# tanmayrainanda/ishara

Hardware: AMD Instinct MI355X
Metric: landmark-frames/sec training (B=256,T=384,d=256) (higher is better)
Workload: dtype bf16; 1 GPU; configs[1]: get_model(dim=256, 2 squeeze + 2 conformer blocks, kernel_sizes=[11,5,3]) CTC train step (fwd+CTC+bwd+RAdam/Lookahead, dropout on); batch_per_gpu=256, global_batch=256, frames=384, features=224, params=7577784, parallelism=dp1, ranks_seen=1

## Files before the change

include/ishara_hip.h:

```cpp
#ifndef ISHARA_HIP_H
#define ISHARA_HIP_H
#include <stdint.h>
#ifdef __cplusplus
extern "C" {
#endif

typedef struct ishara_model ishara_model;
typedef void* ishara_stream;

enum { ISHARA_F32 = 0, ISHARA_BF16 = 1, ISHARA_F16 = 2 };
enum { ISHARA_FAMILY_KERAS_HYBRID = 0, ISHARA_FAMILY_TORCH_CONFORMER = 1, ISHARA_FAMILY_TORCH_SQUEEZEFORMER = 2 };

typedef struct ishara_config {
    int32_t dim;
    int32_t num_conv_squeeze_blocks;
    int32_t num_conv_conform_blocks;
    int32_t num_kernel_sizes;
    int32_t kernel_sizes[8];
    int32_t num_conv_per_block;
    float   dropout_rate;
    int32_t num_heads;
    int32_t expansion_factor;
    int32_t transformer_kernel_size;
    int32_t frames;
// ... 19 lines not shown
int  ishara_create(const ishara_config* cfg, ishara_model** out);
void ishara_destroy(ishara_model* m);

int64_t ishara_param_total(const ishara_model* m);
int64_t ishara_param_trainable(const ishara_model* m);
int32_t ishara_param_entries(const ishara_model* m);
int  ishara_param_info(const ishara_model* m, int32_t i, const char** name, int32_t* ndim,
                       int64_t shape[2], int64_t* offset, int32_t* trainable);
int64_t ishara_workspace_bytes(const ishara_model* m);

int32_t ishara_workspace_plan_check(const ishara_model* m);
int ishara_workspace_guard_check(ishara_model* m);

int ishara_bind(ishara_model* m, float* params, float* grads, float* opt_m, float* opt_v,
                float* opt_slow, void* workspace, int64_t workspace_bytes);
int ishara_sync_weights(ishara_model* m, ishara_stream s);

int ishara_forward(ishara_model* m, const float* x, int32_t B, float* logits, int32_t training,
                   uint32_t seed, ishara_stream s);
int ishara_loss_backward(ishara_model* m, const float* logits, const int64_t* labels, int32_t B,
                         float* loss, float* nll, float loss_scale, ishara_stream s);
int ishara_encoder_forward(ishara_model* m, const float* x, int32_t B, float* y, int32_t training, uint32_t seed, ishara_stream s);
int32_t ishara_encoder_output_frames(const ishara_model* m);
int ishara_encoder_backward(ishara_model* m, const float* dy, int32_t B, float* dx, ishara_stream s);
int32_t ishara_grad_buckets(const ishara_model* m);
int ishara_grad_bucket(const ishara_model* m, int32_t i, int64_t* offset, int64_t* count);
int ishara_grad_buckets_enable(ishara_model* m);
int ishara_grad_bucket_wait(ishara_model* m, int32_t i, ishara_stream side);
int ishara_optimizer_step(ishara_model* m, float lr, float weight_decay, ishara_stream s);
int32_t ishara_optimizer_iterations(const ishara_model* m);
int ishara_optimizer_set_iterations(ishara_model* m, int32_t it);

typedef struct ishara_grad_stats { float norm; float coef; int32_t nonfinite; int32_t skipped; } ishara_grad_stats;
int64_t ishara_grad_stats_workspace_bytes(int64_t n);
int ishara_gradient_stats(ishara_model* prof, const float* g, int64_t n, float grad_scale, float clip_norm, ishara_grad_stats* out, void* ws,
                          ishara_stream s);
int ishara_gradient_accumulate(ishara_model* prof, float* acc, const float* g, int64_t n, int32_t first, ishara_stream s);
int ishara_optimizer_step_ex(ishara_model* m, float lr, float weight_decay, const float* grad, ishara_grad_stats* st, int32_t skip_nonfinite,
                             ishara_stream s);

int ishara_profile_enable(ishara_model* m, int32_t on);
int ishara_profile_report(ishara_model* m, char* buf, int32_t cap);

int ishara_greedy_decode(const float* logits, int32_t B, int32_t T, int32_t C, int32_t blank,
                         int32_t* out_idx, int32_t* out_len, ishara_stream s);
int ishara_preprocess(const float* raw, const int32_t* n_frames, int32_t max_frames, const float* mean, const float* stdv,
                      float* out, int32_t T, ishara_stream s);
int ishara_preprocess_batch(const float* raw, int64_t n_total, const int64_t* offsets, int32_t B, int32_t max_frames,
                            const float* mean, const float* stdv, float* out, int32_t T, ishara_stream s);
int ishara_edit_distance(const int32_t* out_idx, const int32_t* out_len, int32_t B, int32_t T, const int32_t* targets, int32_t L,
                         int32_t* dist, int32_t* tlen, ishara_stream s);

int64_t ishara_ctc_beam_workspace_bytes(int32_t B, int32_t T, int32_t C, int32_t beam_width);
int ishara_ctc_beam_decode(const float* logits, int32_t B, int32_t T, int32_t C, int32_t blank, int32_t beam_width, int32_t nbest,
                           const float* lm, float alpha, float beta, void* workspace,
                           int32_t* out_idx, int32_t* out_len, float* out_score, ishara_stream s);

int64_t ishara_ctc_align_workspace_bytes(int32_t B, int32_t T, int32_t L);
int ishara_ctc_align(const float* logits, const int64_t* labels, int32_t B, int32_t T, int32_t C, int32_t L, int32_t blank,
                     void* ws, int32_t* frame_pos, int32_t* start, int32_t* end, float* conf, float* score, ishara_stream s);

typedef struct ishara_clip_aug {
    int64_t offset;
    int32_t n;
    int32_t L1;
    int32_t shift;
    int32_t L2;
    int32_t mirror;
    int32_t t0[3];
    int32_t t1[3];
    int32_t fingers[3];
} ishara_clip_aug;
enum { ISHARA_LAYOUT_FLAT = 0, ISHARA_LAYOUT_HANDS_LIPS_XY = 1 };
int ishara_clip_batch(const float* raw, const ishara_clip_aug* clips, int32_t B, int32_t T, int32_t layout,
                      float* x, ishara_stream s);
int64_t ishara_ctc_workspace_bytes(int32_t B, int32_t T, int32_t L);
int ishara_ctc_loss(const float* logits, const int64_t* labels, int32_t B, int32_t T, int32_t C,
                    int32_t L, int32_t blank, float* nll, float* dlogits, float grad_scale,
                    void* ws, ishara_stream s);
int ishara_dropout_mask(uint32_t seed, uint32_t site, int32_t rows, int32_t cols, float rate,
                        float* out, ishara_stream s);

int ishara_debug_set_as_flags(int32_t flags);
const char* ishara_debug_dense_kernel_name(int32_t dt, int32_t M, int32_t K, int32_t N, int32_t act, int32_t with_resid);
int ishara_debug_set_nt_big(int32_t on);
int ishara_debug_force_regstage(int32_t on);
int32_t ishara_debug_module_count(ishara_model* m);
int ishara_debug_module_info(ishara_model* m, int32_t i, const char** name, int32_t* in_cols, int32_t* out_cols, int32_t* first_site, int32_t* n_sites);
int ishara_debug_module_forward(ishara_model* m, int32_t i, const float* x, int32_t B, float* y, int32_t training, uint32_t seed, ishara_stream s);
int ishara_debug_module_backward(ishara_model* m, int32_t i, const float* dy, int32_t B, float* dx, ishara_stream s);
int ishara_debug_head_loss_backward(ishara_model* m, const float* logits, const int64_t* labels, int32_t B, float* loss, float* nll,
                                    float loss_scale, float* dx, ishara_stream s);

int64_t ishara_op_scratch_bytes(int32_t M, int32_t K, int32_t N);
int ishara_op_dense_fwd(int32_t dt, const void* x, const float* W, const float* bias, void* y,
                        int32_t M, int32_t K, int32_t N, int32_t act, void* scratch, ishara_stream s);
int ishara_op_dense_fwd_ex(int32_t dt, const void* x, const float* W, const float* bias, const void* resid, void* y,
                           int32_t M, int32_t K, int32_t N, int32_t act, void* scratch, ishara_stream s);
int ishara_op_dense_bwd(int32_t dt, const void* x, const float* W, const void* dy, void* dx,
                        float* dW, float* db, int32_t M, int32_t K, int32_t N, void* scratch, ishara_stream s);
int64_t ishara_op_qkv_scratch_bytes(int32_t B, int32_t T, int32_t H, int32_t dh);
int ishara_op_qkv_fwd(int32_t dt, const void* x, const float* gamma, const float* beta, float eps, const float* W, const float* bias,
                      void* q, void* k, void* vt, int32_t B, int32_t T, int32_t H, int32_t dh, int32_t head_major, void* scratch, ishara_stream s);
int ishara_op_classifier_fwd(int32_t dt, const void* x, const float* W, const float* bias, float* logits, int32_t M, int32_t K, int32_t C,
                             int32_t route, void* scratch, ishara_stream s);
int ishara_op_ctc_loss(const float* logits, const int64_t* labels, int32_t B, int32_t T, int32_t C, int32_t L, int32_t blank,
                       float* nll, float* dlogits, float grad_scale, void* ws, void* dlb, ishara_stream s);
int ishara_op_log_softmax_fwd(const float* x, float* y, int32_t M, int32_t C, int32_t ld, ishara_stream s);
int ishara_op_log_softmax_bwd(const float* dy, const float* y, float* dx, int32_t M, int32_t C, int32_t ld, ishara_stream s);
int ishara_op_layernorm_fwd(int32_t dt, const void* x, const float* gamma, const float* beta, float eps,
                            void* y, float* mean, float* rstd, int32_t M, int32_t C, ishara_stream s);
int ishara_op_layernorm_bwd(int32_t dt, const void* dy, const void* x, const float* mean, const float* rstd,
                            const float* gamma, void* dx, float* dgamma, float* dbeta, int32_t M, int32_t C,
                            ishara_stream s);
int ishara_op_dwconv_fwd(int32_t dt, int32_t inop, const void* x, const float* w, const float* bias, void* y,
                         float* ssum, float* ssq, int32_t B, int32_t T, int32_t C, int32_t k, int32_t padl,
                         ishara_stream s);
int64_t ishara_op_dwconv_fwd_scratch_bytes(int32_t B, int32_t T, int32_t C);
int ishara_op_dwconv_fwd_ex(int32_t dt, int32_t inop, const void* x, const float* w, const float* bias, void* y,
                            float* ssum, float* ssq, void* scratch, int32_t B, int32_t T, int32_t C, int32_t k,
                            int32_t padl, ishara_stream s);
int64_t ishara_op_dwconv_scratch_bytes(int32_t C, int32_t k);
int ishara_op_dwconv_bwd(int32_t dt, int32_t inop, const void* dy, const void* x, const float* w, void* dx,
                         float* dw, float* dbias, void* scratch, int32_t B, int32_t T, int32_t C, int32_t k,
                         int32_t padl, ishara_stream s);
int64_t ishara_op_attn_scratch_bytes(int32_t B, int32_t H, int32_t T, int32_t dh);
int ishara_op_attn_scratch_layout_bytes(int32_t B, int32_t H, int32_t T, int32_t dh, int64_t* out);
int ishara_op_attn_fwd(int32_t dt, const void* qkv, void* o, int32_t B, int32_t H, int32_t T, int32_t dh,
                       float scale, uint32_t seed, uint32_t site, float rate, int32_t impl,
                       void* scratch, ishara_stream s);
int ishara_op_attn_bwd(int32_t dt, const void* o, const void* dout, void* dqkv, int32_t B, int32_t H,
                       int32_t T, int32_t dh, float scale, uint32_t seed, uint32_t site, float rate,
                       int32_t impl, void* scratch, ishara_stream s);

int64_t ishara_op_relattn_scratch_bytes(int32_t B, int32_t H, int32_t T, int32_t dh);
int ishara_op_relattn_fwd(int32_t dt, const void* q, const void* k, const void* v, const float* pe, const float* Wpos, const float* u, const float* vb,
                          void* o, float* lse, int32_t B, int32_t H, int32_t T, int32_t dh, uint32_t seed, uint32_t site, float rate,
                          void* scratch, ishara_stream s);
int ishara_op_relattn_bwd(int32_t dt, const void* q, const void* k, const void* v, const float* u, const float* vb, const void* o, const void* dO,
                          void* dq, void* dk, void* dv, float* du, float* dvb, float* dWpos, float* dposp,
                          int32_t B, int32_t H, int32_t T, int32_t dh, uint32_t seed, uint32_t site, float rate, void* scratch, ishara_stream s);
int64_t ishara_op_r4_subsample_scratch_bytes(int32_t B, int32_t T0, int32_t F, int32_t d);
int ishara_op_r4_subsample_fwd(int32_t dt, const float* x, const float* w1, const float* b1, const float* w2, const float* b2, void* sub,
                               int32_t B, int32_t T0, int32_t F, int32_t d, void* scratch, ishara_stream s);
int ishara_op_r4_subsample_bwd(int32_t dt, const float* x, const float* w1, const float* w2, const void* sub, const void* dsub,
                               float* dw1, float* db1, float* dw2, float* db2, float* dx, int32_t B, int32_t T0, int32_t F, int32_t d,
                               void* scratch, ishara_stream s);
int64_t ishara_op_r4_time_reduce_scratch_bytes(int32_t B, int32_t Tin, int32_t d);
int ishara_op_r4_time_reduce_fwd(int32_t dt, const void* h, const float* conv_w, const float* conv_b, const float* Wred, const float* bred,
                                 void* red, void* conv_out, int32_t B, int32_t Tin, int32_t d, void* scratch, ishara_stream s);
int ishara_op_r4_time_reduce_bwd(int32_t dt, const void* h, const float* conv_w, const void* dred, const void* extra, void* dh,
                                 float* dconv_w, float* dconv_b, float* dWred, float* dbred, int32_t B, int32_t Tin, int32_t d,
                                 void* scratch, ishara_stream s);
int ishara_op_r4_rows(int32_t dt, int32_t mode, const void* src, const void* a, void* dst, int32_t B, int32_t Tdst, int32_t Tsrc, int32_t d,
                      ishara_stream s);

#ifdef __cplusplus
}
#endif
#endif
```

ishara_amd/_lib.py:

```python
from __future__ import annotations

import ctypes as C
import os

_HERE = os.path.dirname(os.path.abspath(__file__))
LIB_PATH = os.path.join(_HERE, "libishara_hip.so")

F32, BF16, F16 = 0, 1, 2
FAMILY_KERAS_HYBRID, FAMILY_TORCH_CONFORMER, FAMILY_TORCH_SQUEEZEFORMER = 0, 1, 2


class IsharaError(RuntimeError):
    pass


class Config(C.Structure):
    _fields_ = [
        ("dim", C.c_int32), ("num_conv_squeeze_blocks", C.c_int32), ("num_conv_conform_blocks", C.c_int32),
        ("num_kernel_sizes", C.c_int32), ("kernel_sizes", C.c_int32 * 8), ("num_conv_per_block", C.c_int32),
        ("dropout_rate", C.c_float), ("num_heads", C.c_int32), ("expansion_factor", C.c_int32),
        ("transformer_kernel_size", C.c_int32), ("frames", C.c_int32), ("features", C.c_int32),
        ("num_classes", C.c_int32), ("top_dim", C.c_int32), ("squeeze_expansion", C.c_int32),
        ("conformer_expansion", C.c_int32), ("head_dropout", C.c_float), ("conformer_attn_dropout", C.c_float),
        ("dtype", C.c_int32), ("max_batch", C.c_int32), ("max_label_len", C.c_int32), ("attn_impl", C.c_int32),
        ("family", C.c_int32), ("reduce_layer_index", C.c_int32), ("recover_layer_index", C.c_int32), ("half_step_residual", C.c_int32),
    ]


class ClipAug(C.Structure):
    _fields_ = [
        ("offset", C.c_int64), ("n", C.c_int32), ("L1", C.c_int32), ("shift", C.c_int32), ("L2", C.c_int32),
        ("mirror", C.c_int32), ("t0", C.c_int32 * 3), ("t1", C.c_int32 * 3), ("fingers", C.c_int32 * 3),
    ]


LAYOUT_FLAT, LAYOUT_HANDS_LIPS_XY = 0, 1


class GradStats(C.Structure):
    _fields_ = [("norm", C.c_float), ("coef", C.c_float), ("nonfinite", C.c_int32), ("skipped", C.c_int32)]


_P, _I32, _I64, _U32, _F = C.c_void_p, C.c_int32, C.c_int64, C.c_uint32, C.c_float
SIGNATURES = {
    "ishara_last_error": (C.c_char_p, []),
    "ishara_create": (C.c_int, [C.POINTER(Config), C.POINTER(_P)]),
    "ishara_destroy": (None, [_P]),
    "ishara_param_total": (_I64, [_P]),
    "ishara_param_trainable": (_I64, [_P]),
    "ishara_param_entries": (_I32, [_P]),
    "ishara_param_info": (C.c_int, [_P, _I32, C.POINTER(C.c_char_p), C.POINTER(_I32), C.POINTER(_I64 * 2), C.POINTER(_I64), C.POINTER(_I32)]),
    "ishara_workspace_bytes": (_I64, [_P]),
    "ishara_workspace_plan_check": (_I32, [_P]),
    "ishara_workspace_guard_check": (C.c_int, [_P]),
    "ishara_grad_buckets": (_I32, [_P]),
    "ishara_grad_bucket": (C.c_int, [_P, _I32, C.POINTER(C.c_int64), C.POINTER(C.c_int64)]),
    "ishara_grad_buckets_enable": (C.c_int, [_P]),
    "ishara_grad_bucket_wait": (C.c_int, [_P, _I32, _P]),
    "ishara_bind": (C.c_int, [_P, _P, _P, _P, _P, _P, _P, _I64]),
    "ishara_sync_weights": (C.c_int, [_P, _P]),
    "ishara_forward": (C.c_int, [_P, _P, _I32, _P, _I32, _U32, _P]),
    "ishara_encoder_forward": (C.c_int, [_P, _P, _I32, _P, _I32, _U32, _P]),
    "ishara_encoder_backward": (C.c_int, [_P, _P, _I32, _P, _P]),
    "ishara_encoder_output_frames": (_I32, [_P]),
    "ishara_loss_backward": (C.c_int, [_P, _P, _P, _I32, _P, _P, _F, _P]),
    "ishara_optimizer_step": (C.c_int, [_P, _F, _F, _P]),
    "ishara_optimizer_iterations": (_I32, [_P]),
    "ishara_optimizer_set_iterations": (C.c_int, [_P, _I32]),
    "ishara_grad_stats_workspace_bytes": (_I64, [_I64]),
    "ishara_gradient_stats": (C.c_int, [_P, _P, _I64, _F, _F, _P, _P, _P]),
    "ishara_gradient_accumulate": (C.c_int, [_P, _P, _P, _I64, _I32, _P]),
    "ishara_optimizer_step_ex": (C.c_int, [_P, _F, _F, _P, _P, _I32, _P]),
    "ishara_profile_enable": (C.c_int, [_P, _I32]),
    "ishara_profile_report": (C.c_int, [_P, C.c_char_p, _I32]),
    "ishara_greedy_decode": (C.c_int, [_P, _I32, _I32, _I32, _I32, _P, _P, _P]),
    "ishara_preprocess": (C.c_int, [_P, _P, _I32, _P, _P, _P, _I32, _P]),
    "ishara_preprocess_batch": (C.c_int, [_P, _I64, _P, _I32, _I32, _P, _P, _P, _I32, _P]),
    "ishara_edit_distance": (C.c_int, [_P, _P, _I32, _I32, _P, _I32, _P, _P, _P]),
    "ishara_ctc_beam_workspace_bytes": (_I64, [_I32, _I32, _I32, _I32]),
    "ishara_ctc_beam_decode": (C.c_int, [_P, _I32, _I32, _I32, _I32, _I32, _I32, _P, _F, _F, _P, _P, _P, _P, _P]),
    "ishara_ctc_align_workspace_bytes": (_I64, [_I32, _I32, _I32]),
    "ishara_ctc_align": (C.c_int, [_P, _P, _I32, _I32, _I32, _I32, _I32, _P, _P, _P, _P, _P, _P, _P]),
    "ishara_clip_batch": (C.c_int, [_P, _P, _I32, _I32, _I32, _P, _P]),
    "ishara_ctc_workspace_bytes": (_I64, [_I32, _I32, _I32]),
    "ishara_ctc_loss": (C.c_int, [_P, _P, _I32, _I32, _I32, _I32, _I32, _P, _P, _F, _P, _P]),
    "ishara_op_ctc_loss": (C.c_int, [_P, _P, _I32, _I32, _I32, _I32, _I32, _P, _P, _F, _P, _P, _P]),
    "ishara_dropout_mask": (C.c_int, [_U32, _U32, _I32, _I32, _F, _P, _P]),
    "ishara_debug_set_as_flags": (C.c_int, [_I32]),
    "ishara_debug_dense_kernel_name": (C.c_char_p, [_I32, _I32, _I32, _I32, _I32, _I32]),
    "ishara_debug_set_nt_big": (C.c_int, [_I32]),
    "ishara_debug_force_regstage": (C.c_int, [_I32]),
    "ishara_debug_module_count": (_I32, [_P]),
    "ishara_debug_module_info": (C.c_int, [_P, _I32, C.POINTER(C.c_char_p), C.POINTER(_I32), C.POINTER(_I32), C.POINTER(_I32), C.POINTER(_I32)]),
    "ishara_debug_module_forward": (C.c_int, [_P, _I32, _P, _I32, _P, _I32, _U32, _P]),
    "ishara_debug_module_backward": (C.c_int, [_P, _I32, _P, _I32, _P, _P]),
    "ishara_debug_head_loss_backward": (C.c_int, [_P, _P, _P, _I32, _P, _P, _F, _P, _P]),
    "ishara_op_scratch_bytes": (_I64, [_I32, _I32, _I32]),
    "ishara_op_dense_fwd": (C.c_int, [_I32, _P, _P, _P, _P, _I32, _I32, _I32, _I32, _P, _P]),
    "ishara_op_dense_fwd_ex": (C.c_int, [_I32, _P, _P, _P, _P, _P, _I32, _I32, _I32, _I32, _P, _P]),
    "ishara_op_dense_bwd": (C.c_int, [_I32, _P, _P, _P, _P, _P, _P, _I32, _I32, _I32, _P, _P]),
    "ishara_op_qkv_scratch_bytes": (_I64, [_I32, _I32, _I32, _I32]),
    "ishara_op_qkv_fwd": (C.c_int, [_I32, _P, _P, _P, _F, _P, _P, _P, _P, _P, _I32, _I32, _I32, _I32, _I32, _P, _P]),
    "ishara_op_classifier_fwd": (C.c_int, [_I32, _P, _P, _P, _P, _I32, _I32, _I32, _I32, _P, _P]),
    "ishara_op_log_softmax_fwd": (C.c_int, [_P, _P, _I32, _I32, _I32, _P]),
    "ishara_op_log_softmax_bwd": (C.c_int, [_P, _P, _P, _I32, _I32, _I32, _P]),
    "ishara_op_layernorm_fwd": (C.c_int, [_I32, _P, _P, _P, _F, _P, _P, _P, _I32, _I32, _P]),
    "ishara_op_layernorm_bwd": (C.c_int, [_I32, _P, _P, _P, _P, _P, _P, _P, _P, _I32, _I32, _P]),
    "ishara_op_dwconv_fwd": (C.c_int, [_I32, _I32, _P, _P, _P, _P, _P, _P, _I32, _I32, _I32, _I32, _I32, _P]),
    "ishara_op_dwconv_scratch_bytes": (_I64, [_I32, _I32]),
    "ishara_op_dwconv_fwd_scratch_bytes": (_I64, [_I32, _I32, _I32]),
    "ishara_op_dwconv_fwd_ex": (C.c_int, [_I32, _I32, _P, _P, _P, _P, _P, _P, _P, _I32, _I32, _I32, _I32, _I32, _P]),
    "ishara_op_dwconv_bwd": (C.c_int, [_I32, _I32, _P, _P, _P, _P, _P, _P, _P, _I32, _I32, _I32, _I32, _I32, _P]),
    "ishara_op_attn_scratch_bytes": (_I64, [_I32, _I32, _I32, _I32]),
    "ishara_op_attn_scratch_layout_bytes": (C.c_int, [_I32, _I32, _I32, _I32, C.POINTER(_I64)]),
    "ishara_op_attn_fwd": (C.c_int, [_I32, _P, _P, _I32, _I32, _I32, _I32, _F, _U32, _U32, _F, _I32, _P, _P]),
    "ishara_op_attn_bwd": (C.c_int, [_I32, _P, _P, _P, _I32, _I32, _I32, _I32, _F, _U32, _U32, _F, _I32, _P, _P]),
    "ishara_op_relattn_scratch_bytes": (_I64, [_I32, _I32, _I32, _I32]),
    "ishara_op_relattn_fwd": (C.c_int, [_I32] + [_P] * 9 + [_I32, _I32, _I32, _I32, _U32, _U32, _F, _P, _P]),
    "ishara_op_relattn_bwd": (C.c_int, [_I32] + [_P] * 14 + [_I32, _I32, _I32, _I32, _U32, _U32, _F, _P, _P]),
    "ishara_op_r4_subsample_scratch_bytes": (_I64, [_I32, _I32, _I32, _I32]),
    "ishara_op_r4_subsample_fwd": (C.c_int, [_I32] + [_P] * 6 + [_I32, _I32, _I32, _I32, _P, _P]),
    "ishara_op_r4_subsample_bwd": (C.c_int, [_I32] + [_P] * 10 + [_I32, _I32, _I32, _I32, _P, _P]),
    "ishara_op_r4_time_reduce_scratch_bytes": (_I64, [_I32, _I32, _I32]),
    "ishara_op_r4_time_reduce_fwd": (C.c_int, [_I32] + [_P] * 7 + [_I32, _I32, _I32, _P, _P]),
    "ishara_op_r4_time_reduce_bwd": (C.c_int, [_I32] + [_P] * 9 + [_I32, _I32, _I32, _P, _P]),
    "ishara_op_r4_rows": (C.c_int, [_I32, _I32, _P, _P, _P, _I32, _I32, _I32, _I32, _P]),
}

_lib = None


def load():
    global _lib
    if _lib is not None:
        return _lib
    if not os.path.exists(LIB_PATH):
        raise IsharaError(f"{LIB_PATH} is missing: build it with `python -m ishara_amd.build` "
                          "(hipcc --offload-arch=gfx950); there is no CPU fallback")
    lib = C.CDLL(LIB_PATH)
    for name, (res, args) in SIGNATURES.items():
        fn = getattr(lib, name)
        fn.restype = res
        fn.argtypes = args
    _lib = lib
    return lib


def check(rc: int, what: str = ""):
    if rc != 0:
        msg = load().ishara_last_error()
        raise IsharaError(f"{what} failed (rc={rc}): {msg.decode() if msg else '?'}")


def ptr(t):
    return None if t is None else C.c_void_p(t.data_ptr())


def stream():
    import torch
    return C.c_void_p(torch.cuda.current_stream().cuda_stream)


def aligned(nbytes: int, device):
    import torch
    t = torch.empty(int(nbytes) + 256, dtype=torch.uint8, device=device)
    return t, C.c_void_p(t.data_ptr() + (-t.data_ptr()) % 256)
```

ishara_amd/csrc/api_ops.hip:

```cpp
#include "model_types.h"

__global__ void dropout_mask_kernel(float* out, int rows, int cols, DropSpec d) {
    const size_t n = (size_t)rows * cols;
    for (size_t i = (size_t)blockIdx.x * blockDim.x + threadIdx.x; i < n; i += (size_t)gridDim.x * blockDim.x) {
        const uint32_t r = (uint32_t)(i / cols), c = (uint32_t)(i % cols);
        out[i] = (d.thr == 0u || rng_keep(rng_row_key(d.key, r), c, d.thr)) ? d.scale : 0.f;
    }
}
template <typename T>
__global__ void qkv_split_kernel(const T* qkv, T* q, T* k, T* vt, int B, int H, int Tn, int dh) {
    const int d = H * dh;
    const size_t n = (size_t)B * Tn * 3 * d;
    for (size_t i = (size_t)blockIdx.x * blockDim.x + threadIdx.x; i < n; i += (size_t)gridDim.x * blockDim.x) {
        const size_t m = i / (3 * d);
        const int col = (int)(i - m * 3 * d);
        const int h = col / (3 * dh), w = col - h * 3 * dh, part = w / dh, e = w - part * dh;
        const int b = (int)(m / Tn), t = (int)(m - (size_t)b * Tn);
        const T v = qkv[i];
        if (part == 0) q[((size_t)(b * H + h) * Tn + t) * dh + e] = v;
        else if (part == 1) k[((size_t)(b * H + h) * Tn + t) * dh + e] = v;
        else vt[((size_t)(b * H + h) * dh + e) * Tn + t] = v;
    }
}

// ... 83 lines not shown
    if (!(alpha == alpha && beta == beta) || alpha - alpha != 0.0f || beta - beta != 0.0f) { ishara_set_error("ishara_ctc_beam_decode: alpha and beta must be finite"); return -1; }
    if (B > 0 && (!logits || !workspace || !out_idx || !out_len || !out_score)) { ishara_set_error("ishara_ctc_beam_decode: null argument"); return -1; }
    if ((uintptr_t)workspace % 4) { ishara_set_error("ishara_ctc_beam_decode: workspace must be 4-byte aligned"); return -1; }
    return launch_ctc_beam(logits, B, T, C, blank, beam_width, nbest, lm, alpha, beta, workspace, out_idx, out_len, out_score, (hipStream_t)s);
}
extern "C" int64_t ishara_ctc_align_workspace_bytes(int32_t B, int32_t T, int32_t L) {
    if (B < 0 || T < 1 || T > 4096 || L < 1 || L > 255) return -1;
    return (int64_t)ctc_align_workspace_bytes(B, T, L);
}
extern "C" int ishara_ctc_align(const float* logits, const int64_t* labels, int32_t B, int32_t T, int32_t C, int32_t L, int32_t blank,
                                void* ws, int32_t* frame_pos, int32_t* start, int32_t* end, float* conf, float* score, ishara_stream s) {
    const char* me = "ishara_ctc_align";
    if (B < 0) { ishara_set_error("%s: B=%d < 0", me, B); return -1; }
    if (T < 1 || T > 4096) { ishara_set_error("%s: T=%d outside 1..4096", me, T); return -1; }
    if (L < 1 || L > 255) { ishara_set_error("%s: L=%d outside 1..255 (2L+1 lattice states in at most 8 registers of a 64-lane wave)", me, L); return -1; }
    if (C < 2 || C > 64) { ishara_set_error("%s: C=%d outside 2..64", me, C); return -1; }
    if (blank < 0 || blank >= C) { ishara_set_error("%s: blank %d outside 0..%d", me, blank, C - 1); return -1; }
    if (B == 0) return 0;
    if (!logits || !labels || !ws || !frame_pos || !start || !end || !conf || !score) {
        ishara_set_error("%s: null logits / labels / ws / frame_pos / start / end / conf / score", me); return -1;
    }
    if ((uintptr_t)ws % 16) { ishara_set_error("%s: ws must be 16-byte aligned", me); return -1; }
    return launch_ctc_align(logits, labels, B, T, C, L, blank, ws, frame_pos, start, end, conf, score, (hipStream_t)s);
}
extern "C" int ishara_clip_batch(const float* raw, const ishara_clip_aug* clips, int32_t B, int32_t T, int32_t layout,
                                 float* x, ishara_stream s) {
    if (B < 0 || T < 1 || T > CLIP_MAX_T) { ishara_set_error("ishara_clip_batch: B=%d T=%d unsupported (B >= 0, 1 <= T <= %d)", B, T, CLIP_MAX_T); return -1; }
    if (layout != ISHARA_LAYOUT_FLAT && layout != ISHARA_LAYOUT_HANDS_LIPS_XY) { ishara_set_error("ishara_clip_batch: unknown layout %d", layout); return -1; }
    if (B > 0 && (!clips || !x)) { ishara_set_error("ishara_clip_batch: null clips / x"); return -1; }
    if (((uintptr_t)raw | (uintptr_t)x) % 16) { ishara_set_error("ishara_clip_batch: raw and x must be 16-byte aligned"); return -1; }
    return launch_clip_batch(raw, clips, B, T, layout, x, (hipStream_t)s);
}

static bool op_dt_ok(const char* op, int dt, bool f16_ok) {
    if (dt != DT_F32 && dt != DT_BF16 && dt != DT_F16) { ishara_set_error("%s: unknown dtype %d (ISHARA_F32 = 0, ISHARA_BF16 = 1, ISHARA_F16 = 2)", op, dt); return false; }
    if (dt == DT_F16 && !f16_ok) { ishara_set_error("%s: ISHARA_F16 is inference-only (no fp16 backward kernels)", op); return false; }
    return true;
}
#define OP_DT(op, dt, f16_ok) do { if (!op_dt_ok(op, dt, f16_ok)) return -1; } while (0)
struct OpShadow {
    size_t wt, wn, slab, total; int ldt, ldn;
    OpShadow(int dt, int K, int N, int M) {
        const int bk = dt_is16(dt) ? 64 : 32;
        const size_t es = dt_size(dt);
        ldt = (int)rup(K, bk); ldn = (int)rup(N, bk);
        wt = 0;
        wn = rup(rup(N, 128) * (size_t)ldt * es, 256);
        slab = wn + rup(rup(K, 128) * (size_t)ldn * es, 256);
        total = slab + gemm_tn_slab_floats(M, K, N, dt) * sizeof(float);
    }
    int build(int dt, const float* Wm, int K, int N, char* sc, hipStream_t s) const {
        HIP_CHECK_RET(hipMemsetAsync(sc, 0, slab, s));
        return launch_make_shadow(dt, Wm, K, N, sc + wt, ldt, sc + wn, ldn, s);
    }
};
extern "C" int64_t ishara_op_scratch_bytes(int32_t M, int32_t K, int32_t N) {
    return (int64_t)OpShadow(DT_F32, K, N, M).total;
}
extern "C" int ishara_op_dense_fwd(int32_t dt, const void* x, const float* Wm, const float* bias, void* y, int32_t M, int32_t K, int32_t N, int32_t act, void* scratch, ishara_stream st) {
    OP_DT("ishara_op_dense_fwd", dt, true);
    hipStream_t s = (hipStream_t)st;
    const OpShadow sh(dt, K, N, M);
    char* sc = (char*)scratch;
    CK(sh.build(dt, Wm, K, N, sc, s));
    OpArgs no; EpiArgs ea; ea.bias = bias; ea.act = act; ea.dbg = g_dbg_epi;
    return launch_gemm_nt(dt, dt, dt, OP_NONE, x, sc + sh.wt, y, M, N, K, sh.ldt, no, ea, s);
}
extern "C" int ishara_op_dense_fwd_ex(int32_t dt, const void* x, const float* Wm, const float* bias, const void* resid, void* y,
                                      int32_t M, int32_t K, int32_t N, int32_t act, void* scratch, ishara_stream st) {
    OP_DT("ishara_op_dense_fwd_ex", dt, true);
    hipStream_t s = (hipStream_t)st;
    const OpShadow sh(dt, K, N, M);
    char* sc = (char*)scratch;
    CK(sh.build(dt, Wm, K, N, sc, s));
    OpArgs no; EpiArgs ea; ea.bias = bias; ea.act = act; ea.resid = resid; ea.dbg = g_dbg_epi;
    return launch_gemm_nt(dt, dt, dt, OP_NONE, x, sc + sh.wt, y, M, N, K, sh.ldt, no, ea, s);
}
extern "C" const char* ishara_debug_dense_kernel_name(int32_t dt, int32_t M, int32_t K, int32_t N, int32_t act, int32_t with_resid) {
    if (!op_dt_ok("ishara_debug_dense_kernel_name", dt, true) || M < 1 || K < 1 || N < 1) return "";
    const OpShadow sh(dt, K, N, M);
    const void* aligned = reinterpret_cast<const void*>(uintptr_t(256));
    EpiArgs ea; ea.bias = reinterpret_cast<const float*>(aligned); ea.act = act; ea.resid = with_resid ? aligned : nullptr; ea.dbg = g_dbg_epi;
    return gemm_nt_kernel_name(dt, dt, dt, OP_NONE, aligned, M, N, K, sh.ldt, ea);
}
extern "C" int ishara_op_dense_bwd(int32_t dt, const void* x, const float* Wm, const void* dy, void* dx, float* dW, float* db,
                                   int32_t M, int32_t K, int32_t N, void* scratch, ishara_stream st) {
    OP_DT("ishara_op_dense_bwd", dt, false);
    hipStream_t s = (hipStream_t)st;
    const OpShadow sh(dt, K, N, M);
    char* sc = (char*)scratch;
    CK(sh.build(dt, Wm, K, N, sc, s));
    OpArgs no; EpiArgs ea;
    if (dx) CK(launch_gemm_nt(dt, dt, dt, OP_NONE, dy, sc + sh.wn, dx, M, K, N, sh.ldn, no, ea, s));
    return launch_gemm_tn(dt, dt, dt, OP_NONE, OP_NONE, x, dy, dW, db, (float*)(sc + sh.slab), M, K, N, no, no, s);
}
static void qkv_scratch_layout(int B, int T, int H, int dh, size_t& xn, size_t& mean, size_t& rstd, size_t& total) {
    const int M = B * T, d = H * dh;
    xn = rup(OpShadow(DT_F32, d, 3 * d, M).total, 256);
    mean = xn + rup((size_t)M * d * 4, 256);
    rstd = mean + rup((size_t)M * 4, 256);
    total = rstd + rup((size_t)M * 4, 256);
}
extern "C" int64_t ishara_op_qkv_scratch_bytes(int32_t B, int32_t T, int32_t H, int32_t dh) {
    if (B < 1 || T < 1 || H < 1 || dh < 1) return -1;
    size_t xn, mean, rstd, total;
    qkv_scratch_layout(B, T, H, dh, xn, mean, rstd, total);
    return (int64_t)total;
}
extern "C" int ishara_op_qkv_fwd(int32_t dt, const void* x, const float* gamma, const float* beta, float eps, const float* Wm, const float* bias,
                                 void* q, void* k, void* vt, int32_t B, int32_t T, int32_t H, int32_t dh, int32_t head_major, void* scratch, ishara_stream st) {
    OP_DT("ishara_op_qkv_fwd", dt, true);
    if (B < 1 || T < 1 || H < 1 || dh < 1 || T % 8 != 0 || dh % 8 != 0 || (head_major != 0 && head_major != 1)) {
        ishara_set_error("ishara_op_qkv_fwd: B=%d T=%d H=%d dh=%d head_major=%d unsupported (T, dh multiples of 8; head_major 0 / 1)", B, T, H, dh, head_major); return -1;
    }
    const int d = H * dh, M = B * T;
    if ((gamma != nullptr) != (beta != nullptr) || (gamma && d > 512)) { ishara_set_error("ishara_op_qkv_fwd: LayerNorm needs both gamma and beta and H*dh <= 512 (H*dh=%d)", d); return -1; }
    if (!x || !Wm || !q || !k || !vt || !scratch || ((uintptr_t)x | (uintptr_t)scratch) % 16 != 0) { ishara_set_error("ishara_op_qkv_fwd: null or misaligned buffer (x, scratch: 16-byte aligned)"); return -1; }
    hipStream_t s = (hipStream_t)st;
    const OpShadow sh(dt, d, 3 * d, M);
    char* sc = (char*)scratch;
    CK(sh.build(dt, Wm, d, 3 * d, sc, s));
    OpArgs no;
    EpiArgs eq; eq.mode = EPI_QKV; eq.q = q; eq.k = k; eq.vt = vt; eq.H = H; eq.dh = dh; eq.T = T; eq.head_major = head_major;
    const void* A = x;
    if (gamma && !ln_as_prologue(dt, M, 3 * d, d, sh.ldt, gamma, beta, eps, nullptr, nullptr, nullptr, eq)) {
        size_t xn, mean, rstd, tot;
        qkv_scratch_layout(B, T, H, dh, xn, mean, rstd, tot);
        CK(launch_layernorm_fwd(dt, x, gamma, beta, eps, sc + xn, (float*)(sc + mean), (float*)(sc + rstd), M, d, s));
        A = sc + xn;
    }
    eq.bias = bias;
    return launch_gemm_nt(dt, dt, dt, OP_NONE, A, sc + sh.wt, nullptr, M, 3 * d, d, sh.ldt, no, eq, s);
}
extern "C" int ishara_op_classifier_fwd(int32_t dt, const void* x, const float* Wm, const float* bias, float* logits, int32_t M, int32_t K, int32_t C,
                                        int32_t route, void* scratch, ishara_stream st) {
    OP_DT("ishara_op_classifier_fwd", dt, true);
    if (route < CLS_AUTO || route > CLS_GEMM) { ishara_set_error("ishara_op_classifier_fwd: unknown route %d (0 auto, 1 A-stationary, 2 dense_narrow, 3 GEMM)", route); return -1; }
    if (M < 1 || K < 1 || C < 1) { ishara_set_error("ishara_op_classifier_fwd: bad shape M=%d K=%d C=%d", M, K, C); return -1; }
    const int r = route == CLS_AUTO ? cls_route_auto(dt, M, K, C) : route;
    const char* why = nullptr;
    if (r != CLS_GEMM && !dt_is16(dt)) why = "16-bit operands only";
    else if (r == CLS_AS && (C > 64 || C % 4 != 0 || (K != 256 && K != 512))) why = "C <= 64, C % 4 == 0 and K 256 / 512 only";
    else if (r == CLS_AS && g_force_regstage) why = "the A-stationary kernel is switched off (ishara_debug_force_regstage)";
    else if (r == CLS_NARROW && (C > 64 || K % 32 != 0)) why = "C <= 64 and K % 32 == 0 only";
    else if (r == CLS_GEMM && K % (dt_is16(dt) ? 8 : 4) != 0) why = "16-byte operand rows only";
    if (why) { ishara_set_error("ishara_op_classifier_fwd: route %d does not take dt=%d M=%d K=%d C=%d: %s", r, dt, M, K, C, why); return -1; }
    if (!x || !Wm || !logits || !scratch || ((uintptr_t)x | (uintptr_t)scratch) % 16 != 0) { ishara_set_error("ishara_op_classifier_fwd: null or misaligned buffer (x, scratch: 16-byte aligned)"); return -1; }
    hipStream_t s = (hipStream_t)st;
    const OpShadow sh(dt, K, C, M);
    char* sc = (char*)scratch;
    CK(sh.build(dt, Wm, K, C, sc, s));
    return classifier_fwd(nullptr, r, dt, x, sc + sh.wt, sh.ldt, bias, logits, M, K, C, s);
}
extern "C" int ishara_op_log_softmax_fwd(const float* x, float* y, int32_t M, int32_t C, int32_t ld, ishara_stream s) { return launch_log_softmax_fwd(x, y, M, C, ld, (hipStream_t)s); }
extern "C" int ishara_op_log_softmax_bwd(const float* dy, const float* y, float* dx, int32_t M, int32_t C, int32_t ld, ishara_stream s) { return launch_log_softmax_bwd(dy, y, dx, M, C, ld, (hipStream_t)s); }
extern "C" int ishara_op_layernorm_fwd(int32_t dt, const void* x, const float* gamma, const float* beta, float eps, void* y, float* mean, float* rstd, int32_t M, int32_t C, ishara_stream s) {
    OP_DT("ishara_op_layernorm_fwd", dt, true);
    return launch_layernorm_fwd(dt, x, gamma, beta, eps, y, mean, rstd, M, C, (hipStream_t)s);
}
extern "C" int ishara_op_layernorm_bwd(int32_t dt, const void* dy, const void* x, const float* mean, const float* rstd, const float* gamma, void* dx, float* dgamma, float* dbeta, int32_t M, int32_t C, ishara_stream s) {
    OP_DT("ishara_op_layernorm_bwd", dt, false);
    return launch_layernorm_bwd(dt, dy, x, mean, rstd, gamma, nullptr, dx, dgamma, dbeta, nullptr, M, C, (hipStream_t)s);
}
extern "C" int ishara_op_dwconv_fwd(int32_t dt, int32_t inop, const void* x, const float* w, const float* bias, void* y, float* ssum, float* ssq,
                                    int32_t B, int32_t T, int32_t C, int32_t k, int32_t padl, ishara_stream s) {
    OP_DT("ishara_op_dwconv_fwd", dt, true);
// ... 268 lines not shown
```

ishara_amd/csrc/gemm_cs.hip:

```cpp
#include <cstdio>
#include <cstdlib>
#include <map>
#include "common.h"
#include "kernels.h"

enum { CS_RESID = 1, CS_DROP = 8, CS_ROWSCALE = 16 };
#define CS_K 512
#define CS_N 256
#define CS_ROWS 384
#define CS_NST 8
#define CS_RING 4
#define CS_STAGE 32768
#define CS_DPW 4
#define CS_LDS (CS_RING * CS_STAGE + CS_N * 4 + 2 * CS_K * 4)
#define CS_DEFAULT_FLAGS 115
#define CS_MIN_M 49153

typedef __attribute__((ext_vector_type(4))) uint32_t cs_u32x4;

template <int N> DEVI void cs_wait_vm() { static_assert(N >= 0 && N < 64, "vmcnt is 6 bits"); asm volatile("s_waitcnt vmcnt(%0)" ::"n"(N) : "memory"); }
template <int N0, int NP> DEVI void cs_wait(bool counted, bool pout) {
    if (!counted) cs_wait_vm<0>(); else if (pout) cs_wait_vm<NP>(); else cs_wait_vm<N0>();
}
template <int OFF> DEVI cs_u32x4 cs_ld16(const void* p) {
    cs_u32x4 r;
    asm volatile("global_load_dwordx4 %0, %1, off offset:%2" : "=v"(r) : "v"(p), "n"(OFF) : "memory");
    return r;
}
DEVI void cs_pin(cs_u32x4& r) { asm volatile("" : "+v"(r)); }
DEVI void cs_mfma(bool first, f32x4& acc, const bf16x8& b, const cs_u32x4& a) {
    if (first) asm volatile("v_mfma_f32_16x16x32_bf16 %0, %1, %2, 0" : "=&v"(acc) : "v"(b), "v"(a));
    else asm volatile("v_mfma_f32_16x16x32_bf16 %0, %1, %2, %0" : "+v"(acc) : "v"(b), "v"(a));
}
DEVI int cs_swz(int r) { return (r & 2) | (((r >> 4) & 1) << 2); }
DEVI void cs_unpack(const cs_u32x4& r, float (&v)[8]) {
#pragma unroll
    for (int h = 0; h < 4; ++h) { v[2 * h] = __uint_as_float(r[h] << 16); v[2 * h + 1] = __uint_as_float(r[h] & 0xffff0000u); }
}
DEVI void cs_st_pk(bf16* p, const bf16x8& t, bool nt) {
    if (nt) __builtin_nontemporal_store(t, reinterpret_cast<bf16x8*>(p)); else *reinterpret_cast<bf16x8*>(p) = t;
}

struct CsLane {
    const bf16* bsrc[CS_DPW];
    int off0, off1;
    int wid, c, g;
};
template <int RT> struct CsRows {
    const bf16* ap[RT];
    int mrow[RT];
    cs_u32x4 a[3][RT][2];
};
template <int RT> DEVI void cs_rows_init(CsRows<RT>& r, const bf16* __restrict__ A, int M, int mw, const CsLane& L) {
#pragma unroll
    for (int i = 0; i < RT; ++i) {
        r.mrow[i] = min(mw + 16 * i + L.c, M - 1);
        r.ap[i] = A + (size_t)r.mrow[i] * CS_K + L.g * 8;
    }
}
template <int RT, int S> DEVI void cs_load_a(CsRows<RT>& r) {
#pragma unroll
    for (int i = 0; i < RT; ++i) {
        r.a[S % 3][i][0] = cs_ld16<S * 128>(r.ap[i]);
        r.a[S % 3][i][1] = cs_ld16<S * 128 + 64>(r.ap[i]);
    }
}
template <int S> DEVI void cs_issue_w(const CsLane& L, char* smem) {
#pragma unroll
    for (int t = 0; t < CS_DPW; ++t) {
        const bf16* src = L.bsrc[t];
        asm volatile("" : "+v"(src));
        __builtin_amdgcn_global_load_lds((const __attribute__((address_space(1))) void*)(src + S * 64),
                                         (__attribute__((address_space(3))) void*)(smem + (S % CS_RING) * CS_STAGE + (L.wid * CS_DPW + t) * 1024), 16, 0, 0);
    }
}
template <int RT> DEVI void cs_prefetch(CsRows<RT>& r, const CsLane& L, char* smem) {
    cs_load_a<RT, 0>(r);
    cs_load_a<RT, 1>(r);
    cs_issue_w<0>(L, smem);
    cs_issue_w<1>(L, smem);
    cs_issue_w<2>(L, smem);
}
#define CS_PREFETCH_OPS(RT) (2 * 2 * (RT) + 3 * CS_DPW)

template <int MASK, int PRO, int RT, int E, int S>
DEVI void cs_stage(CsRows<RT>& r, const CsLane& L, char* smem, const float* pq_s, f32x4 (&acc)[8][2][RT], bf16* pro_out, int M, int mw,
                   bool full, bool pout, bool nt_side) {
    constexpr int NA = 2 * RT, D = CS_DPW;
    if constexpr (S == 0) cs_wait<2 * D + E, 2 * D + E>(full, pout);
    else if constexpr (S == 1) cs_wait<2 * D + E + NA, 2 * D + E + NA + NA>(full, pout);
    else if constexpr (S <= 5) cs_wait<2 * D + NA, 2 * D + NA + 2 * NA>(full, pout);
    else if constexpr (S == 6) cs_wait<D + NA, D + NA + 2 * NA>(full, pout);
    else cs_wait<0, 2 * NA>(full, pout);
    asm volatile("s_waitcnt lgkmcnt(0)" ::: "memory");
    __builtin_amdgcn_s_barrier();
    if constexpr (S + 2 < CS_NST) cs_load_a<RT, S + 2>(r);
    if constexpr (S + 3 < CS_NST) cs_issue_w<S + 3>(L, smem);
    constexpr int B = S % 3;
#pragma unroll
    for (int i = 0; i < RT; ++i) { cs_pin(r.a[B][i][0]); cs_pin(r.a[B][i][1]); }
    if constexpr (PRO == 2) {
#pragma unroll
        for (int kt = 0; kt < 2; ++kt) {
            const float* cp = pq_s + 64 * S + 32 * kt + 8 * L.g;
            const f32x4 w0 = *reinterpret_cast<const f32x4*>(cp), w1 = *reinterpret_cast<const f32x4*>(cp + 4);
            const f32x4 b0 = *reinterpret_cast<const f32x4*>(cp + CS_K), b1 = *reinterpret_cast<const f32x4*>(cp + CS_K + 4);
            float wv[8], bv[8];
#pragma unroll
            for (int e = 0; e < 4; ++e) { wv[e] = w0[e]; wv[4 + e] = w1[e]; bv[e] = b0[e]; bv[4 + e] = b1[e]; }
#pragma unroll
            for (int i = 0; i < RT; ++i) {
                float v[8];
                cs_unpack(r.a[B][i][kt], v);
                bf16x8 t;
#pragma unroll
                for (int e = 0; e < 8; ++e) t[e] = (bf16)(v[e] * wv[e] + bv[e]);
                r.a[B][i][kt] = __builtin_bit_cast(cs_u32x4, t);
                if (pout && (full || mw + 16 * i + L.c < M))
                    cs_st_pk(pro_out + (size_t)r.mrow[i] * CS_K + L.g * 8 + 64 * S + 32 * kt, t, nt_side);
            }
        }
    }
    const char* st = smem + (S % CS_RING) * CS_STAGE;
    auto frag = [&](int q, int jj) { return *reinterpret_cast<const bf16x8*>(st + ((q >> 3) ? L.off1 : L.off0) + (32 * (q & 7) + 4 * jj) * 128); };
    bf16x8 b0 = frag(0, 0), b1 = frag(0, 1), c0 = frag(1, 0), c1 = frag(1, 1);
    if constexpr (PRO != 0) asm volatile("s_nop 1");
#pragma unroll
    for (int q = 0; q < 16; ++q) {
        const int kt = q >> 3, p = q & 7;
        bf16x8 n0 = c0, n1 = c1;
        if (q + 2 < 16) { n0 = frag(q + 2, 0); n1 = frag(q + 2, 1); }
        asm volatile("" ::: "memory");
#pragma unroll
        for (int i = 0; i < RT; ++i) {
            cs_mfma(S == 0 && q < 8, acc[p][0][i], b0, r.a[B][i][kt]);
            cs_mfma(S == 0 && q < 8, acc[p][1][i], b1, r.a[B][i][kt]);
        }
        b0 = c0; b1 = c1; c0 = n0; c1 = n1;
    }
}

template <int MASK, int PRO, int RT, int E, typename HAND>
DEVI void cs_pass(CsRows<RT>& r, const CsLane& L, bf16* __restrict__ C, int M, const EpiArgs& ea, char* smem, const float* bias_s, const float* pq_s,
                  int m_base, float rsc, int hops, HAND hand) {
    const int mw = m_base + L.wid * 16 * RT;
    const bool full = m_base + 128 * RT <= M;
    const bool pout = PRO != 0 && ea.pro_out != nullptr;
    const bool nt_side = (ea.as_flags & 2) != 0;
    constexpr bool f_resid = (MASK & CS_RESID) != 0, f_drop = (MASK & CS_DROP) != 0, f_rowscale = (MASK & CS_ROWSCALE) != 0;
    f32x4 acc[8][2][RT];
    bf16* po = reinterpret_cast<bf16*>(ea.pro_out);
    cs_stage<MASK, PRO, RT, E, 0>(r, L, smem, pq_s, acc, po, M, mw, full, pout, nt_side);
    cs_stage<MASK, PRO, RT, E, 1>(r, L, smem, pq_s, acc, po, M, mw, full, pout, nt_side);
    cs_stage<MASK, PRO, RT, E, 2>(r, L, smem, pq_s, acc, po, M, mw, full, pout, nt_side);
    cs_stage<MASK, PRO, RT, E, 3>(r, L, smem, pq_s, acc, po, M, mw, full, pout, nt_side);
    cs_stage<MASK, PRO, RT, E, 4>(r, L, smem, pq_s, acc, po, M, mw, full, pout, nt_side);
    cs_stage<MASK, PRO, RT, E, 5>(r, L, smem, pq_s, acc, po, M, mw, full, pout, nt_side);
    cs_stage<MASK, PRO, RT, E, 6>(r, L, smem, pq_s, acc, po, M, mw, full, pout, nt_side);
    cs_stage<MASK, PRO, RT, E, 7>(r, L, smem, pq_s, acc, po, M, mw, full, pout, nt_side);

    asm volatile("s_nop 15");
    size_t eoff[RT];
#pragma unroll
    for (int i = 0; i < RT; ++i) eoff[i] = (size_t)r.mrow[i] * CS_N + 8 * L.g;
    cs_u32x4 rs[RT][8];
    if constexpr (f_resid) {
        const bf16* resid = reinterpret_cast<const bf16*>(ea.resid);
#pragma unroll
        for (int i = 0; i < RT; ++i) {
            const bf16* rp = resid + eoff[i];
            rs[i][0] = cs_ld16<0>(rp);   rs[i][1] = cs_ld16<64>(rp);  rs[i][2] = cs_ld16<128>(rp); rs[i][3] = cs_ld16<192>(rp);
            rs[i][4] = cs_ld16<256>(rp); rs[i][5] = cs_ld16<320>(rp); rs[i][6] = cs_ld16<384>(rp); rs[i][7] = cs_ld16<448>(rp);
        }
    }
    asm volatile("s_waitcnt lgkmcnt(0)" ::: "memory");
    __builtin_amdgcn_s_barrier();
    hand();
    if constexpr (f_resid) {
        if (hops) cs_wait_vm<CS_PREFETCH_OPS(1)>(); else cs_wait_vm<0>();
#pragma unroll
        for (int i = 0; i < RT; ++i)
#pragma unroll
            for (int p = 0; p < 8; ++p) cs_pin(rs[i][p]);
    }
    uint32_t rk[RT];
#pragma unroll
    for (int i = 0; i < RT; ++i) rk[i] = f_drop ? rng_row_key(ea.drop.key, (uint32_t)(mw + 16 * i + L.c)) : 0u;
#pragma unroll
    for (int i = 0; i < RT; ++i) {
        const int m = mw + 16 * i + L.c;
        if (!full && m >= M) continue;
#pragma unroll
        for (int p = 0; p < 8; ++p) {
            const int n = 32 * p + 8 * L.g;
            float bias[8];
#pragma unroll
            for (int h = 0; h < 2; ++h) {
                const f32x4 bv = *reinterpret_cast<const f32x4*>(bias_s + n + 4 * h);
#pragma unroll
                for (int e = 0; e < 4; ++e) bias[4 * h + e] = bv[e];
            }
            float v[8];
            const float bsc = (f_rowscale && ea.rowscale_bias) ? rsc : 1.f;
#pragma unroll
            for (int e = 0; e < 4; ++e) { v[e] = acc[p][0][i][e] + bias[e] * bsc; v[4 + e] = acc[p][1][i][e] + bias[4 + e] * bsc; }
            if constexpr (f_drop) rng_apply<8>(rk[i], (uint32_t)n, ea.drop.thr, ea.drop.scale, v);
            if (f_rowscale && !ea.rowscale_bias) {
#pragma unroll
                for (int e = 0; e < 8; ++e) v[e] *= rsc;
            }
            if constexpr (f_resid) {
                float x[8];
                cs_unpack(rs[i][p], x);
#pragma unroll
                for (int e = 0; e < 8; ++e) v[e] += x[e];
            }
            store8(C + eoff[i] + 32 * p, v);
        }
    }
}

template <int MASK, int PRO>
__global__ __launch_bounds__(512, 1) void gemm_nt_cs_kernel(const bf16* __restrict__ A, const bf16* __restrict__ Bt, bf16* __restrict__ C, int M, int ldb, EpiArgs ea) {
    extern __shared__ __attribute__((aligned(16))) char cs_smem[];
    float* bias_s = reinterpret_cast<float*>(cs_smem + CS_RING * CS_STAGE);
    float* pq_s = bias_s + CS_N;
    const int tid = threadIdx.x, lane = tid & 63;
    const int m_base = blockIdx.x * CS_ROWS;
    const int bsm = min(m_base, M - 1) / max(ea.T, 1);
    for (int n = tid; n < CS_N; n += 512) bias_s[n] = ea.bias ? ea.bias[n] : 0.f;
    if constexpr (PRO == 2) {
        const float* c0 = ea.pa_P + (size_t)bsm * CS_K;
        const float* c1 = ea.pa_Q + (size_t)bsm * CS_K;
        for (int x = tid; x < CS_K; x += 512) { pq_s[x] = c0[x]; pq_s[CS_K + x] = c1[x]; }
    }
    float rsc = 1.f;
    if constexpr ((MASK & CS_ROWSCALE) != 0) rsc = ea.rowscale[bsm];
    __syncthreads();
    asm volatile("" : "+v"(rsc));

    CsLane L;
    L.wid = __builtin_amdgcn_readfirstlane(tid >> 6);
    L.c = lane & 15; L.g = lane >> 4;
#pragma unroll
    for (int t = 0; t < CS_DPW; ++t) {
        const int rr = (L.wid * CS_DPW + t) * 8 + (lane >> 3), p = lane & 7;
        L.bsrc[t] = Bt + (size_t)rr * ldb + ((p ^ cs_swz(rr)) << 3);
    }
    const int frow = 8 * (L.c >> 2) + (L.c & 3);
    const int sx = L.g ^ cs_swz(frow);
    L.off0 = frow * 128 + (sx << 4);
    L.off1 = frow * 128 + ((sx ^ 4) << 4);

    const bool two = m_base + 256 < M;
    CsRows<2> r1;
    CsRows<1> r2;
    cs_rows_init<2>(r1, A, M, m_base + L.wid * 32, L);
    cs_prefetch<2>(r1, L, cs_smem);
    cs_pass<MASK, PRO, 2, 0>(r1, L, C, M, ea, cs_smem, bias_s, pq_s, m_base, rsc, two ? CS_PREFETCH_OPS(1) : 0, [&]() {
        if (two) {
            cs_rows_init<1>(r2, A, M, m_base + 256 + L.wid * 16, L);
            cs_prefetch<1>(r2, L, cs_smem);
        }
    });
    if (two) cs_pass<MASK, PRO, 1, 16>(r2, L, C, M, ea, cs_smem, bias_s, pq_s, m_base + 256, rsc, 0, []() {});
}

static int cs_mask_of(const EpiArgs& ea) {
    return (ea.resid ? 1 : 0) | (ea.dact != DACT_NONE ? 2 : 0) | (ea.act != ACT_NONE ? 4 : 0) | (ea.drop.thr ? 8 : 0) | (ea.rowscale ? 16 : 0) |
           (ea.pre_out ? 32 : 0) | (ea.mode == EPI_QKV ? 64 : 0) | (ea.addtab ? 128 : 0);
}
static int cs_flags(const EpiArgs& ea) {
    static const int v = getenv("ISHARA_AS_FLAGS") ? atoi(getenv("ISHARA_AS_FLAGS")) : CS_DEFAULT_FLAGS;
    return ea.as_flags >= 0 ? ea.as_flags : (g_as_flags_override >= 0 ? g_as_flags_override : v);
}
bool gemm_nt_cs_applicable(int dtC, int M, int N, int K, int ldb, const EpiArgs& ea) {
    if (dtC != DT_BF16 || K != CS_K || N != CS_N || M < 1 || ldb < CS_K || ldb % 8 != 0) return false;
    const int flags = cs_flags(ea);
    if (!(flags & 64)) return false;
    if (ea.n_valid || ea.dbg || (ea.ldc && ea.ldc != CS_N) || ea.ln_gamma) return false;
    if (!(flags & 128) && M < CS_MIN_M) return false;
    const int mask = cs_mask_of(ea);
    if (ea.pa_P) return ea.pa_Q && ea.T > 0 && ea.T % CS_ROWS == 0 && (mask == CS_RESID || mask == (CS_RESID | CS_ROWSCALE));
    return mask == 0 || mask == CS_RESID || mask == (CS_RESID | CS_DROP);
}
const char* gemm_nt_cs_name(const EpiArgs& ea) {
    static std::map<int, std::string> names;
    const int mask = cs_mask_of(ea), pro = ea.pa_P ? 2 : 0;
    auto it = names.find(mask | pro << 8);
    if (it == names.end()) {
        char buf[64];
        snprintf(buf, sizeof buf, "gemm_nt_cs_kernel<%d,%d>", mask, pro);
        it = names.emplace(mask | pro << 8, buf).first;
    }
    return it->second.c_str();
}
template <int MASK, int PRO>
static int cs_launch(const void* A, const void* Bt, void* C, int M, int ldb, const EpiArgs& ea, hipStream_t s) {
    static int ready = 0;
    if (!ready) ready = hipFuncSetAttribute(reinterpret_cast<const void*>(gemm_nt_cs_kernel<MASK, PRO>), hipFuncAttributeMaxDynamicSharedMemorySize, CS_LDS) == hipSuccess ? 1 : -1;
    if (ready < 0) { ishara_set_error("gemm_nt_cs: %d bytes of LDS refused", CS_LDS); return -1; }
    hipLaunchKernelGGL((gemm_nt_cs_kernel<MASK, PRO>), dim3((M + CS_ROWS - 1) / CS_ROWS), dim3(512), CS_LDS, s, (const bf16*)A, (const bf16*)Bt, (bf16*)C, M, ldb, ea);
    return launch_rc();
}
int launch_gemm_nt_cs(int dtC, const void* A, const void* Bt, void* C, int M, int N, int K, int ldb, const EpiArgs& ea_in, hipStream_t s) {
    if (!gemm_nt_cs_applicable(dtC, M, N, K, ldb, ea_in)) return 1;
    EpiArgs ea = ea_in;
    ea.as_flags = cs_flags(ea_in);
    const int mask = cs_mask_of(ea);
    if (ea.pa_P) return mask == CS_RESID ? cs_launch<CS_RESID, 2>(A, Bt, C, M, ldb, ea, s) : cs_launch<CS_RESID | CS_ROWSCALE, 2>(A, Bt, C, M, ldb, ea, s);
    if (mask == 0) return cs_launch<0, 0>(A, Bt, C, M, ldb, ea, s);
    if (mask == CS_RESID) return cs_launch<CS_RESID, 0>(A, Bt, C, M, ldb, ea, s);
    return cs_launch<CS_RESID | CS_DROP, 0>(A, Bt, C, M, ldb, ea, s);
}
```

ishara_amd/csrc/gemm_nt.hip:

```cpp
#include "gemm_tile.h"

template <typename TA, typename TM, typename TC, int OP>
__global__ __launch_bounds__(256) void gemm_nt_kernel(const TA* __restrict__ A, const TM* __restrict__ Bt, TC* __restrict__ C,
                                                      int M, int N, int K, int ldb, int a_vec_ok, OpArgs oa, EpiArgs ea) {
    __shared__ __attribute__((aligned(16))) char smem[65536];
    constexpr int BK = MmaCfg<TM>::BK;
    const int tid = threadIdx.x, lane = tid & 63, wid = tid >> 6, wr = wid >> 1, wc = wid & 1;
    const int nMt = (M + 127) >> 7, nNt = (N + 127) >> 7;
    int mt, nt;
    {
        const int id = blockIdx.x;
        if ((nMt & 7) == 0) { const int xcd = id & 7, local = id >> 3; mt = (local / nNt) * 8 + xcd; nt = local % nNt; }
        else { mt = id / nNt; nt = id % nNt; }
    }
    const int m0 = mt << 7, n0 = nt << 7;
    const int nk = (K + BK - 1) / BK;

    u32x4 ra[4], rb[4];
    f32x4 acc[4][4];
#pragma unroll
    for (int i = 0; i < 4; ++i)
#pragma unroll
        for (int j = 0; j < 4; ++j) acc[i][j] = f32x4{0.f, 0.f, 0.f, 0.f};

// ... 413 lines not shown
                    if (ea.rowscale && !ea.rowscale_bias) {
#pragma unroll
                        for (int e = 0; e < 4; ++e) v[e] *= rsc;
                    }
                    if (need_aux) {
                        float a4[4];
                        if (need_res) load4t(reinterpret_cast<const TC*>(ea.aux) + rowoff + n, a4);
                        else {
#pragma unroll
                            for (int e = 0; e < 4; ++e) a4[e] = ext[j][e];
                        }
                        if (ea.dact == DACT_SWISH) {
#pragma unroll
                            for (int e = 0; e < 4; ++e) v[e] *= dswishf_(a4[e]);
                        } else {
#pragma unroll
                            for (int e = 0; e < 4; ++e) v[e] = a4[e] > 0.f ? v[e] : 0.f;
                        }
                    }
                    if (need_res) {
#pragma unroll
                        for (int e = 0; e < 4; ++e) v[e] += ext[j][e];
                    }
                    if (ea.mode == EPI_STD) {
                        store4t(C + rowoff + n, v);
                    } else {
                        int h, part, ii;
                        if (ea.head_major) { h = n / (3 * ea.dh); const int w = n - h * 3 * ea.dh; part = w / ea.dh; ii = w - part * ea.dh; }
                        else { part = n / dmodel; const int w = n - part * dmodel; h = w / ea.dh; ii = w - h * ea.dh; }
                        const int t = m - bsamp * ea.T;
                        if (part < 2) {
                            store4t(reinterpret_cast<TC*>(part == 0 ? ea.q : ea.k) + ((size_t)(bsamp * ea.H + h) * ea.T + t) * ea.dh + ii, v);
                        } else {
                            TC* dst = reinterpret_cast<TC*>(ea.vt) + ((size_t)(bsamp * ea.H + h) * ea.dh + ii) * ea.T + t;
#pragma unroll
                            for (int e = 0; e < 4; ++e) dst[(size_t)e * ea.T] = from_f<TC>(v[e]);
                        }
                    }
                }
            }
        } else if (acc[0][0][0] == 123.456f) C[0] = from_f<TC>(acc[1][3][2]);
        if (!more) break;
        tile = ntile; mt = mt2; nt = nt2; first = false;
    }
}

template <typename TM, typename TC>
static int run_nt_t(const void* A, const void* Bt, void* C, int M, int N, int K, int ldb, const EpiArgs& ea, hipStream_t s) {
    const int nMt = (M + 127) / 128, nNt = (N + 127) / 128;
    const int ntiles = nMt * nNt;
    const int grid = ntiles < 768 ? ntiles : 768;
    const bool fast = ea.addtab == nullptr && ea.pre_out == nullptr && ea.act == ACT_NONE && ea.drop.thr == 0 && ea.rowscale == nullptr &&
                      ea.dact == DACT_NONE && ea.mode == EPI_STD && ea.dbg == 0;
    if (fast && ea.resid) hipLaunchKernelGGL((gemm_nt_t_kernel<TM, TC, 2>), dim3(grid), dim3(256), 0, s, (const TM*)A, (const TM*)Bt, (TC*)C, M, N, K, ldb, ea);
    else if (fast) hipLaunchKernelGGL((gemm_nt_t_kernel<TM, TC, 1>), dim3(grid), dim3(256), 0, s, (const TM*)A, (const TM*)Bt, (TC*)C, M, N, K, ldb, ea);
    else hipLaunchKernelGGL((gemm_nt_t_kernel<TM, TC, 0>), dim3(grid), dim3(256), 0, s, (const TM*)A, (const TM*)Bt, (TC*)C, M, N, K, ldb, ea);
    return launch_rc();
}

template <typename TA, typename TM, typename TC, int OP>
static int run_nt(const void* A, const void* Bt, void* C, int M, int N, int K, int ldb, const OpArgs& oa, const EpiArgs& ea, hipStream_t s) {
    const int nMt = (M + 127) / 128, nNt = (N + 127) / 128;
    const int a_vec_ok = (((size_t)K * sizeof(TA)) % 16 == 0) && (((uintptr_t)A) % 16 == 0);
    hipLaunchKernelGGL((gemm_nt_kernel<TA, TM, TC, OP>), dim3(nMt * nNt), dim3(256), 0, s,
                       (const TA*)A, (const TM*)Bt, (TC*)C, M, N, K, ldb, a_vec_ok, oa, ea);
    return launch_rc();
}

template <typename TA, typename TM, typename TC>
static int run_nt_op(int op, const void* A, const void* Bt, void* C, int M, int N, int K, int ldb, const OpArgs& oa, const EpiArgs& ea, hipStream_t s) {
    switch (op) {
        case OP_NONE: return run_nt<TA, TM, TC, OP_NONE>(A, Bt, C, M, N, K, ldb, oa, ea, s);
        case OP_SWISH: return run_nt<TA, TM, TC, OP_SWISH>(A, Bt, C, M, N, K, ldb, oa, ea, s);
        case OP_COLAFFINE: return run_nt<TA, TM, TC, OP_COLAFFINE>(A, Bt, C, M, N, K, ldb, oa, ea, s);
        case OP_DROPMASK: return run_nt<TA, TM, TC, OP_DROPMASK>(A, Bt, C, M, N, K, ldb, oa, ea, s);
        default: ishara_set_error("gemm_nt: unsupported operand op %d", op); return -1;
    }
}

int g_force_regstage = 0;

NtRoute gemm_nt_route(int dtA, int dtM, int dtC, int op, const void* A, int M, int N, int K, int ldb, const EpiArgs& ea) {
    const bool pro = ea.ln_gamma || ea.pa_P;
    if (dtM == DT_F16) {
        if (op != OP_NONE) return NT_REFUSED;
        if (dtA == DT_F16 && g_force_regstage == 0 && (K == 256 || K == 512) && ldb % 64 == 0 && ((uintptr_t)A) % 16 == 0 && gemm_nt_as_applicable(dtC, M, N, K, ldb, ea)) return NT_AS_F16;
        if (pro) return NT_REFUSED;
        return (dtA == DT_F16 && (dtC == DT_F16 || dtC == DT_F32)) || (dtA == DT_F32 && dtC == DT_F16) ? NT_REG : NT_REFUSED;
    }
    if (pro && (op != OP_NONE || !gemm_nt_as_prologue_ok(dtA, dtM, dtC, M, N, K, ldb, ea))) return NT_REFUSED;
    if (g_force_regstage == 0 && gemm_nt_big_applicable(dtA, dtM, dtC, op, A, M, N, K, ldb, ea)) return NT_BIG;
    const int bk = dtM == DT_BF16 ? 32 : 16;
    const bool dma_ok = op == OP_NONE && dtA == dtM && K % bk == 0 && ldb % (2 * bk) == 0 && ((uintptr_t)A) % 16 == 0;
    if (dma_ok && g_force_regstage == 0 && dtM == DT_BF16 && gemm_nt_cs_applicable(dtC, M, N, K, ldb, ea)) return NT_CS;
    if (dma_ok && g_force_regstage == 0 && dtM == DT_BF16 && gemm_nt_as_applicable(dtC, M, N, K, ldb, ea)) return NT_AS;
    const bool dma_dt = (dtM == DT_F32 && dtC == DT_F32) || (dtM == DT_BF16 && (dtC == DT_BF16 || dtC == DT_F32));
    if (dma_ok && dma_dt && (g_force_regstage == 0 || g_force_regstage == 3) && N % 4 == 0 && (ea.mode != EPI_QKV || ea.dh % 4 == 0)) return NT_TILE_T;
    if (dma_ok && dma_dt && g_force_regstage != 1) return NT_GLDS;
    if (dtA == dtM && dtM == dtC && (dtM == DT_F32 || dtM == DT_BF16)) return NT_REG;
    if (dtM == DT_BF16 && op == OP_NONE && ((dtA == DT_F32 && dtC == DT_BF16) || (dtA == DT_BF16 && dtC == DT_F32))) return NT_REG;
    return NT_REFUSED;
}

int launch_gemm_nt(int dtA, int dtM, int dtC, int op, const void* A, const void* Bt, void* C,
                   int M, int N, int K, int ldb, const OpArgs& oa, const EpiArgs& ea, hipStream_t s) {
    if (M <= 0 || N <= 0 || K <= 0) { ishara_set_error("gemm_nt: bad shape %d %d %d", M, N, K); return -1; }
    if ((dt_is16(dtA) && K % 8 != 0) || (dtA == DT_F32 && K % 4 != 0) || ((uintptr_t)A) % 16 != 0) {
        ishara_set_error("gemm_nt: A rows must be 16-byte aligned (K=%d)", K); return -1;
    }
    if (ea.mode == EPI_QKV && (ea.T % 8 != 0 || N % 8 != 0 || ea.dh % 8 != 0)) {
        ishara_set_error("gemm_nt: QKV split needs T, dh multiples of 8 (T=%d dh=%d)", ea.T, ea.dh); return -1;
    }
    const bool f16m = dtM == DT_F16;
    int rc = 1;
    switch (gemm_nt_route(dtA, dtM, dtC, op, A, M, N, K, ldb, ea)) {
        case NT_REFUSED:
            if (f16m && op != OP_NONE) ishara_set_error("gemm_nt: f16 operands take no operand transform");
            else if (f16m && (ea.ln_gamma || ea.pa_P)) ishara_set_error("gemm_nt: f16 operand prologue on a shape the A-stationary kernel does not take");
            else if (f16m) ishara_set_error("gemm_nt: unsupported f16 dtype combination %d/%d/%d", dtA, dtM, dtC);
            else if (ea.ln_gamma || ea.pa_P) ishara_set_error("gemm_nt: operand prologue requested for a shape the A-stationary kernel does not take (check gemm_nt_as_prologue_ok first)");
            else ishara_set_error("gemm_nt: unsupported dtype combination %d/%d/%d op %d", dtA, dtM, dtC, op);
            return -1;
        case NT_AS_F16: rc = launch_gemm_nt_as_f16(dtC, A, Bt, C, M, N, K, ldb, ea, s); break;
        case NT_BIG: rc = launch_gemm_nt_big(dtA, dtM, dtC, op, A, Bt, C, M, N, K, ldb, ea, s); break;
        case NT_CS: rc = launch_gemm_nt_cs(dtC, A, Bt, C, M, N, K, ldb, ea, s); break;
        case NT_AS: rc = launch_gemm_nt_as(dtC, A, Bt, C, M, N, K, ldb, ea, s); break;
        case NT_TILE_T:
            if (dtM == DT_F32) return run_nt_t<float, float>(A, Bt, C, M, N, K, ldb, ea, s);
            return dtC == DT_BF16 ? run_nt_t<bf16, bf16>(A, Bt, C, M, N, K, ldb, ea, s) : run_nt_t<bf16, float>(A, Bt, C, M, N, K, ldb, ea, s);
        case NT_GLDS:
            if (dtM == DT_F32) return run_nt_glds<float, float>(A, Bt, C, M, N, K, ldb, ea, s);
            return dtC == DT_BF16 ? run_nt_glds<bf16, bf16>(A, Bt, C, M, N, K, ldb, ea, s) : run_nt_glds<bf16, float>(A, Bt, C, M, N, K, ldb, ea, s);
        case NT_REG:
            if (f16m && dtA == DT_F32) return run_nt<float, f16, f16, OP_NONE>(A, Bt, C, M, N, K, ldb, oa, ea, s);
            if (f16m) return dtC == DT_F16 ? run_nt<f16, f16, f16, OP_NONE>(A, Bt, C, M, N, K, ldb, oa, ea, s) : run_nt<f16, f16, float, OP_NONE>(A, Bt, C, M, N, K, ldb, oa, ea, s);
            if (dtA != dtM) return run_nt<float, bf16, bf16, OP_NONE>(A, Bt, C, M, N, K, ldb, oa, ea, s);
            if (dtC != dtM) return run_nt<bf16, bf16, float, OP_NONE>(A, Bt, C, M, N, K, ldb, oa, ea, s);
            return dtM == DT_F32 ? run_nt_op<float, float, float>(op, A, Bt, C, M, N, K, ldb, oa, ea, s) : run_nt_op<bf16, bf16, bf16>(op, A, Bt, C, M, N, K, ldb, oa, ea, s);
    }
    if (rc == 1) { ishara_set_error("gemm_nt: internal error: the kernel gemm_nt_route chose refused the call (M=%d N=%d K=%d)", M, N, K); return -1; }
    return rc;
}

const char* gemm_nt_kernel_name(int dtA, int dtM, int dtC, int op, const void* A, int M, int N, int K, int ldb, const EpiArgs& ea) {
    const NtRoute route = gemm_nt_route(dtA, dtM, dtC, op, A, M, N, K, ldb, ea);
    if (dtM == DT_F16) return "gemm_nt_kernel<f16>";
    switch (route) {
        case NT_BIG: return "gemm_nt_big_kernel<bf16>";
        case NT_CS: return gemm_nt_cs_name(ea);
        case NT_AS: return gemm_nt_as_name(dtC, K, ea, M, N);
        case NT_TILE_T: return dtM == DT_F32 ? "gemm_nt_t_kernel<f32,f32>" : (dtC == DT_F32 ? "gemm_nt_t_kernel<bf16,f32>" : "gemm_nt_t_kernel<bf16,bf16>");
        case NT_GLDS: return dtM == DT_F32 ? "gemm_nt_glds_kernel<f32,f32>" : (dtC == DT_F32 ? "gemm_nt_glds_kernel<bf16,f32>" : "gemm_nt_glds_kernel<bf16,bf16>");
        default: break;
    }
    if (dtA == DT_F32 && dtM == DT_BF16) return "gemm_nt_kernel<f32,bf16,bf16>";
    if (dtM == DT_F32) return "gemm_nt_kernel<f32,f32,f32>";
    return dtC == DT_F32 ? "gemm_nt_kernel<bf16,bf16,f32>" : "gemm_nt_kernel<bf16,bf16,bf16>";
}
```

ishara_amd/csrc/keras_hybrid.hip:

```cpp
#include "model_types.h"
#include <stdlib.h>

__global__ void droppath_kernel(float* rs, int B, DropSpec d) {
    const int b = blockIdx.x * blockDim.x + threadIdx.x;
    if (b < B) rs[b] = (d.thr == 0u || rng_keep(rng_row_key(d.key, (uint32_t)b), 0u, d.thr)) ? d.scale : 0.f;
}

static void build_conv(ishara_model* m, const std::string& name, int k) {
    ConvBlock cb;
    const int d = m->d, c = 2 * d;
    cb.k = k;
    cb.W1 = m->dense(name + "_expand_conv", d, c, true);
    cb.dw = m->addp(name + "_dwconv/depthwise_kernel", k, c, true);
    cb.bn = m->bnp(name + "_bn", c);
    cb.eca = m->addp(name + "_eca/kernel", 5, 0, true);
    cb.W2 = m->dense(name + "_project_conv", c, d, true);
    cb.site = m->nsites++;
    m->convs.push_back(cb);
    m->layers.push_back({Layer::CONV, (int)m->convs.size() - 1});
    m->layer_entry_end.push_back(m->entries.size());
}
static FFN build_ffn(ishara_model* m, Norm ln, float eps, const std::string& n1, const std::string& n2, int e, bool out_drop) {
    FFN f; f.ln = ln; f.eps = eps;
    f.Wa = m->dense(n1, m->d, m->d * e, true);
// ... 398 lines not shown
        return -1;
    }
    m->s = (hipStream_t)st;
    Run r{B, B * m->T, training, seed};
    CK(stem_fwd(m, r, x));
    const void* h = m->W(m->stem_out);
    for (const Layer& L : m->layers) {
        if (L.kind == Layer::CONV) { ConvBlock& cb = m->convs[L.idx]; CK(conv_fwd(m, cb, r, h)); h = m->W(cb.out); }
        else if (L.kind == Layer::SQZ) {
            SqzBlock& sb = m->sqz[L.idx];
            CK(ffn_fwd(m, sb.ffn1, r, h)); h = m->W(sb.ffn1.out);
            CK(mhsa_fwd(m, sb.mha, r, h)); h = m->W(sb.mha.out);
            CK(sqzconv_fwd(m, sb.conv, r, h)); h = m->W(sb.conv.out);
            CK(ffn_fwd(m, sb.ffn2, r, h)); h = m->W(sb.ffn2.out);
        } else {
            ConfBlock& cb = m->conf[L.idx];
            CK(ffn_fwd(m, cb.ffn1, r, h)); h = m->W(cb.ffn1.out);
            CK(mhsa_fwd(m, cb.mha, r, h)); h = m->W(cb.mha.out);
            CK(confconv_fwd(m, cb.conv, r, h)); h = m->W(cb.conv.out);
            CK(ffn_fwd(m, cb.ffn2, r, h)); h = m->W(cb.ffn2.out);
        }
    }
    CK(head_fwd(m, r, h, logits));
    m->lastB = B; m->last_training = training; m->last_seed = seed; m->last_x = x; m->probe_mod = -1;
    return 0;
}

static const void* layer_out(ishara_model* m, const Layer& L) {
    return L.kind == Layer::CONV ? m->W(m->convs[L.idx].out) : (L.kind == Layer::SQZ ? m->W(m->sqz[L.idx].ffn2.out) : m->W(m->conf[L.idx].ffn2.out));
}
static int conv_bwd(ishara_model* m, ConvBlock& cb, const Run& r, const void* x, const void* g, void* gn) {
    const int d = m->d, c = 2 * d, B = r.B, T = m->T, dt = m->dt;
    OpArgs no;
    const DropSpec ds = dspec(r, cb.site, m->cfg.dropout_rate);
    const void* gs = g;
    EpiArgs e1;
    if (cb.psa) {
        const float* rs = ds.thr ? m->Wf(cb.rs) : nullptr;
        if (rs) { e1.rowscale = rs; e1.T = T; }
        CK(gemm_dgrad(m, cb.W2, g, dt, m->W(m->t1), r.M, OP_NONE, no, e1));
        TnPsa ps; ps.P = m->Wf(cb.P); ps.Q = m->Wf(cb.Q); ps.W = m->ws + cb.W2.wn; ps.ldw = cb.W2.ldn; ps.G = m->Wf(m->psaG); ps.Rpart = m->Wf(m->psaR); ps.T = T;
        { static const int psa_dbg = getenv("ISHARA_PSA_DBG") ? atoi(getenv("ISHARA_PSA_DBG")) : 0; ps.dbg = psa_dbg; }
        CK(gemm_wgrad(m, cb.W2, m->W(cb.h2), dt, OP_NONE, no, g, dt, OP_NONE, no, r.M, 0, 0, rs, rs ? T : 0, &ps));
    } else if (ds.thr && cb.folded) {
        e1.rowscale = m->Wf(cb.rs); e1.T = T;
        CK(gemm_dgrad(m, cb.W2, g, dt, m->W(m->t1), r.M, OP_NONE, no, e1));
        CK(gemm_wgrad(m, cb.W2, m->W(cb.h4), dt, OP_NONE, no, g, dt, OP_NONE, no, r.M, 0, 0, m->Wf(cb.rs), T));
    } else {
        if (ds.thr) {
            CKP(m, "map_rows", 2.0 * r.M * d * (double)dt_size(m->dt), 0, launch_map_rows(dt, MAP_ROWSCALE, g, m->W(m->t3), m->Wf(cb.rs), ds, r.M, T, d, m->s));
            gs = m->W(m->t3);
        }
        CK(gemm_dgrad(m, cb.W2, gs, dt, m->W(m->t1), r.M, OP_NONE, no, e1));
        CK(gemm_wgrad(m, cb.W2, m->W(cb.h4), dt, OP_NONE, no, gs, dt, OP_NONE, no, r.M));
    }
    if (!cb.psa) CKP(m, "sample_reduce", 2.0 * r.M * m->d * (double)dt_size(m->dt), 0, launch_sample_reduce(dt, m->W(m->t1), m->W(cb.h2), m->Wf(cb.mean), m->Wf(cb.rstd), m->Wf(m->S1), m->Wf(m->S2), B, T, c, m->s));
    PsaStats pst;
    if (cb.psa) { pst.G = m->Wf(m->psaG); pst.Rpart = m->Wf(m->psaR); pst.nparts = cb.W2.N / 64; pst.Wt = m->ws + cb.W2.wt; pst.ldt = cb.W2.ldt; pst.N = cb.W2.N;
                  pst.rs = ds.thr ? m->Wf(cb.rs) : nullptr; pst.mean = m->Wf(cb.mean); pst.rstd = m->Wf(cb.rstd); }
    CKP(m, "eca_bn_bwd_finalize", 0, 0, launch_eca_bn_bwd_finalize(m->Wf(m->S1), m->Wf(m->S2), m->Wf(cb.ssum), m->Wf(cb.gn), m->Wf(cb.sg), m->P(cb.eca), m->P(cb.bn.gamma), m->P(cb.bn.beta),
                                  m->Wf(cb.mean), m->Wf(cb.rstd), m->G(cb.bn.gamma), m->G(cb.bn.beta), m->G(cb.eca), m->Wf(m->E), m->Wf(m->Fc), m->Wf(m->ecap), B, T, c, m->s, cb.psa ? &pst : nullptr));
    DwBnArgs bn; bn.h = m->W(cb.h2); bn.mean = m->Wf(cb.mean); bn.rstd = m->Wf(cb.rstd); bn.a = m->Wf(cb.a); bn.sg = m->Wf(cb.sg); bn.E = m->Wf(m->E); bn.Fc = m->Wf(m->Fc); bn.e_per_sample = 1;
    const int fused = dwconv_bwd_deferred(m, r, 10.0, DWIN_SWISH, m->W(m->t1), &bn, m->W(cb.z1), cb.dw, -1, m->W(m->t2), c, cb.k, cb.k - 1);
    if (fused < 0) return fused;
    if (!fused) {
        CKP(m, "bn_bwd_apply", 6.0 * r.M * m->d * (double)dt_size(m->dt), 0, launch_bn_bwd_apply(dt, m->W(m->t1), m->W(cb.h2), m->Wf(cb.mean), m->Wf(cb.rstd), m->Wf(cb.a), m->Wf(cb.sg), m->Wf(m->E), 1, m->Wf(m->Fc), m->W(m->t1), B, T, c, m->s));
        CK(dwconv_bwd_deferred(m, r, 8.0, DWIN_SWISH, m->W(m->t1), nullptr, m->W(cb.z1), cb.dw, -1, m->W(m->t2), c, cb.k, cb.k - 1));
    }
    EpiArgs e2; e2.resid = g;
    CK(gemm_dgrad(m, cb.W1, m->W(m->t2), dt, gn, r.M, OP_NONE, no, e2));
    CK(gemm_wgrad(m, cb.W1, x, dt, OP_NONE, no, m->W(m->t2), dt, OP_NONE, no, r.M));
    return 0;
}

static int ffn_bwd(ishara_model* m, FFN& f, const Run& r, const void* x, const void* g, void* gn) {
    const int dt = m->dt;
    OpArgs no;
    int rc = 0;
    const void* gs = f.has_out_drop ? grad_through_dropout(m, r, f.site_out, m->cfg.dropout_rate, g, m->W(m->t3), m->T, m->d, &rc) : g;
    CK(rc);
    EpiArgs e1; e1.drop = dspec(r, f.site_in, m->cfg.dropout_rate); e1.dact = DACT_SWISH; e1.aux = m->W(f.za);
    CK(gemm_dgrad(m, f.Wb, gs, dt, m->W(m->t1), r.M, OP_NONE, no, e1));
    CK(gemm_wgrad(m, f.Wb, m->W(f.u), dt, OP_NONE, no, gs, dt, OP_NONE, no, r.M));
    EpiArgs e0;
    CK(gemm_dgrad(m, f.Wa, m->W(m->t1), dt, m->W(m->t2), r.M, OP_NONE, no, e0));
    CK(gemm_wgrad(m, f.Wa, m->W(f.xn), dt, OP_NONE, no, m->W(m->t1), dt, OP_NONE, no, r.M));
    return layernorm_bwd_deferred(m, r, m->W(m->t2), x, f.mean, f.rstd, f.ln, g, gn);
}

static int mhsa_bwd(ishara_model* m, MHSA& a, const Run& r, const void* x, const void* g, void* gn) {
    const int dt = m->dt;
    OpArgs no; EpiArgs e0;
    int rc = 0;
    const void* gs = a.has_out_drop ? grad_through_dropout(m, r, a.site_out, m->cfg.dropout_rate, g, m->W(m->t3), m->T, m->d, &rc) : g;
    CK(rc);
    CK(gemm_dgrad(m, a.Wp, gs, dt, m->W(m->t1), r.M, OP_NONE, no, e0));
    CK(gemm_wgrad(m, a.Wp, m->W(a.o), dt, OP_NONE, no, gs, dt, OP_NONE, no, r.M));
    const float scale = 1.0f / sqrtf((float)m->d);
    CKP(m, "attn_bwd", 8.0 * r.M * m->d * (double)dt_size(m->dt), 10.0 * r.B * m->H * (double)m->T * m->T * m->dh, launch_attn_bwd(dt, m->W(a.q), m->W(a.k), m->W(a.vt), m->W(a.o), m->W(m->t1), m->Wf(a.lse), m->Wf(m->delta), m->W(m->t2),
                       r.B, m->H, m->T, m->dh, scale, dspec_attn(r, a.site_attn, a.rate), 1, m->cfg.attn_impl, attn_maskw(m, a.maskw), m->s));
    CK(gemm_dgrad(m, a.Wqkv, m->W(m->t2), dt, m->W(m->t1), r.M, OP_NONE, no, e0));
    CK(gemm_wgrad(m, a.Wqkv, m->W(a.xn), dt, OP_NONE, no, m->W(m->t2), dt, OP_NONE, no, r.M));
    return layernorm_bwd_deferred(m, r, m->W(m->t1), x, a.mean, a.rstd, a.ln, g, gn);
}

static int sqzconv_bwd(ishara_model* m, SqzConv& c, const Run& r, const void* x, const void* g, void* gn) {
    const int dt = m->dt, d = m->d, de = c.Wc1.N, B = r.B, T = m->T;
    OpArgs no; EpiArgs e0;
    CKP(m, "sample_reduce", 2.0 * r.M * m->d * (double)dt_size(m->dt), 0, launch_sample_reduce(dt, g, m->W(c.u3), nullptr, nullptr, m->Wf(m->S1), m->Wf(m->dse), B, T, d, m->s));
    CKP(m, "se_bwd", 0, 0, launch_se_bwd(m->Wf(m->dse), m->Wf(c.gap), 1.f / T, m->P(c.seW1), m->P(c.seW2), m->Wf(c.hid), m->Wf(c.se),
                     m->G(c.seW1), m->G(c.seb1), m->G(c.seW2), m->G(c.seb2), m->Wf(m->dgapT), m->Wf(m->E), B, d, c.R, m->s));
    CKP(m, "sample_affine", 4.0 * r.M * m->d * (double)dt_size(m->dt), 0, launch_sample_affine(dt, g, m->Wf(c.se), m->Wf(m->dgapT), nullptr, m->W(m->t1), B, T, d, m->s));
    EpiArgs e1; e1.dact = DACT_SWISH; e1.aux = m->W(c.zd);
    CK(gemm_dgrad(m, c.Wc3, m->W(m->t1), dt, m->W(m->t2), r.M, OP_NONE, no, e1));
    CK(gemm_wgrad(m, c.Wc3, m->W(c.hd), dt, OP_NONE, no, m->W(m->t1), dt, OP_NONE, no, r.M));
    CK(dwconv_bwd_deferred(m, r, 8.0, DWIN_SWISH, m->W(m->t2), nullptr, m->W(c.zc), c.dw, -1, m->W(m->t1), de, c.k, c.k - 1));
    CK(gemm_dgrad(m, c.Wc1, m->W(m->t1), dt, m->W(m->t2), r.M, OP_NONE, no, e0));
    CK(gemm_wgrad(m, c.Wc1, m->W(c.xn), dt, OP_NONE, no, m->W(m->t1), dt, OP_NONE, no, r.M));
    return layernorm_bwd_deferred(m, r, m->W(m->t2), x, c.mean, c.rstd, c.ln, g, gn);
}

int confconv_bwd(ishara_model* m, ConfConv& c, const Run& r, const void* x, const void* g, void* gn) {
    const int dt = m->dt, d = m->d, B = r.B, T = m->T;
    OpArgs no;
    CK(layernorm_bwd_deferred(m, r, g, m->W(c.r), c.lnmean, c.lnrstd, c.ln, nullptr, m->W(m->t1)));
    int rc = 0;
    const void* gs = c.has_out_drop ? grad_through_dropout(m, r, c.site_out, m->cfg.dropout_rate, m->W(m->t1), m->W(m->t3), T, d, &rc) : m->W(m->t1);
    CK(rc);
    EpiArgs es; if (c.swish_after_bn) { es.dact = DACT_SWISH; es.aux = m->W(c.bnv); }
    CK(gemm_dgrad(m, c.Wp2, gs, dt, m->W(m->t2), r.M, OP_NONE, no, es));
    CK(gemm_wgrad(m, c.Wp2, c.swish_after_bn ? m->W(c.sw) : m->W(c.bnv), dt, OP_NONE, no, gs, dt, OP_NONE, no, r.M));
    CKP(m, "sample_reduce", 2.0 * r.M * m->d * (double)dt_size(m->dt), 0, launch_sample_reduce(dt, m->W(m->t2), m->W(c.v), m->Wf(c.mean), m->Wf(c.rstd), m->Wf(m->S1), m->Wf(m->S2), B, T, d, m->s));
    CKP(m, "bn_bwd_finalize", 0, 0, launch_bn_bwd_finalize(m->Wf(m->S1), m->Wf(m->S2), m->G(c.bn.gamma), m->G(c.bn.beta), m->Wf(m->Ecol), m->Wf(m->Fc), B, T, d, m->s));
    DwBnArgs bn; bn.h = m->W(c.v); bn.mean = m->Wf(c.mean); bn.rstd = m->Wf(c.rstd); bn.a = m->Wf(c.a); bn.E = m->Wf(m->Ecol); bn.Fc = m->Wf(m->Fc);
    const int fused = dwconv_bwd_deferred(m, r, 6.0, DWIN_GLU, m->W(m->t2), &bn, m->W(c.g), c.dw, c.dwb, m->W(m->t3), d, c.k, (c.k - 1) / 2);
    if (fused < 0) return fused;
    if (!fused) {
        CKP(m, "bn_bwd_apply", 6.0 * r.M * m->d * (double)dt_size(m->dt), 0, launch_bn_bwd_apply(dt, m->W(m->t2), m->W(c.v), m->Wf(c.mean), m->Wf(c.rstd), m->Wf(c.a), nullptr, m->Wf(m->Ecol), 0, m->Wf(m->Fc), m->W(m->t2), B, T, d, m->s));
        CK(dwconv_bwd_deferred(m, r, 8.0, DWIN_GLU, m->W(m->t2), nullptr, m->W(c.g), c.dw, c.dwb, m->W(m->t3), d, c.k, (c.k - 1) / 2));
    }
    EpiArgs e2; e2.resid = m->W(m->t1);
    CK(gemm_dgrad(m, c.Wp1, m->W(m->t3), dt, gn, r.M, OP_NONE, no, e2));
    CK(gemm_wgrad(m, c.Wp1, x, dt, OP_NONE, no, m->W(m->t3), dt, OP_NONE, no, r.M));
    return 0;
}

static int head_bwd(ishara_model* m, const Run& r, const void* hin, void* g) {
    const int dt = m->dt;
    OpArgs no; EpiArgs e0;
    EpiArgs eh; eh.drop = dspec(r, m->head_site, m->cfg.head_dropout); eh.dact = DACT_POS; eh.aux = m->W(m->head_hh);
    if (m->cls_pad && r.M % 64 == 0 && r.M >= 256 && m->clsW.K % 128 == 0 && !g_force_tn_regstage) {
        DenseW wp = m->clsW; wp.N = m->cls_pad;
        CK(gemm_dgrad(m, wp, m->W(m->dlb), dt, m->W(m->t1), r.M, OP_NONE, no, eh));
        CK(gemm_wgrad(m, wp, m->W(m->head_hh), dt, OP_NONE, no, m->W(m->dlb), dt, OP_NONE, no, r.M, 0, m->C));
    } else {
        CK(gemm_dgrad(m, m->clsW, m->Wf(m->dlogits), DT_F32, m->W(m->t1), r.M, OP_NONE, no, eh));
        CK(gemm_wgrad(m, m->clsW, m->W(m->head_hh), dt, OP_NONE, no, m->Wf(m->dlogits), DT_F32, OP_NONE, no, r.M));
    }
    CK(gemm_dgrad(m, m->topW, m->W(m->t1), dt, g, r.M, OP_NONE, no, e0));
    CK(gemm_wgrad(m, m->topW, hin, dt, OP_NONE, no, m->W(m->t1), dt, OP_NONE, no, r.M));
    return 0;
}
static int stem_bwd(ishara_model* m, const Run& r, const void* g) {
    const int dt = m->dt, d = m->d, T = m->T, B = r.B;
    OpArgs no;
    CKP(m, "sample_reduce", 2.0 * r.M * m->d * (double)dt_size(m->dt), 0, launch_sample_reduce(dt, g, m->W(m->stem_h0), m->Wf(m->stem_mean), m->Wf(m->stem_rstd), m->Wf(m->S1), m->Wf(m->S2), B, T, d, m->s));
    CKP(m, "bn_bwd_finalize", 0, 0, launch_bn_bwd_finalize(m->Wf(m->S1), m->Wf(m->S2), m->G(m->stem_bn.gamma), m->G(m->stem_bn.beta), m->Wf(m->Ecol), m->Wf(m->Fc), B, T, d, m->s));
    CKP(m, "bn_bwd_apply", 6.0 * r.M * m->d * (double)dt_size(m->dt), 0, launch_bn_bwd_apply(dt, g, m->W(m->stem_h0), m->Wf(m->stem_mean), m->Wf(m->stem_rstd), m->Wf(m->stem_a), nullptr, m->Wf(m->Ecol), 0, m->Wf(m->Fc), m->W(m->t1), B, T, d, m->s));
    if (m->stem_kp && r.M % 64 == 0 && r.M >= 256 && d % 128 == 0 && !g_force_tn_regstage) {
        DenseW wp = m->stemW; wp.K = m->stem_kp;
        CK(gemm_wgrad(m, wp, m->W(m->stem_xb), dt, OP_NONE, no, m->W(m->t1), dt, OP_NONE, no, r.M, m->F));
    } else
        CK(gemm_wgrad(m, m->stemW, m->last_x, DT_F32, OP_NONE, no, m->W(m->t1), dt, OP_NONE, no, r.M));
    return 0;
}

extern "C" int ishara_loss_backward(ishara_model* m, const float* logits, const int64_t* labels, int32_t B, float* loss, float* nll, float loss_scale, ishara_stream st) {
    if (!m->ws || !m->grads) { ishara_set_error("ishara_loss_backward: model is not bound (grads required)"); return -1; }
    if (m->family != ISHARA_FAMILY_KERAS_HYBRID) { ishara_set_error("ishara_loss_backward: this handle is an encoder-only family; use ishara_encoder_backward"); return -1; }
    if (B != m->lastB || !m->last_training) { ishara_set_error("ishara_loss_backward: call ishara_forward(training=1) with the same batch first"); return -1; }
    m->s = (hipStream_t)st;
    m->red.njobs = 0; m->red.nblocks = 0; m->red_off = 0; g_red_sink = nullptr;
    m->tn_defer.pending = false;
    Run r{B, B * m->T, 1, m->last_seed};
    const int T = m->T;
    float* nl = nll ? nll : m->Wf(m->nllb);
    CK(launch_fill_u32(m->grads, (size_t)m->n_train, 0u, m->s));
    CKP(m, "ctc", 2.0 * r.M * m->C * 4, 0, launch_ctc(logits, labels, B, T, m->C, m->L, m->C - 1, nl, m->Wf(m->dlogits), loss_scale / (float)B, m->Wf(m->ctcws), m->s, m->cls_pad ? m->W(m->dlb) : nullptr));
    if (loss) CKP(m, "mean", 0, 0, launch_mean(nl, loss, B, 1.f / (float)B, m->s));
    const void* hin = m->layers.empty() ? m->W(m->stem_out) : layer_out(m, m->layers.back());
    void* g = m->W(m->gA); void* gn = m->W(m->gB);
    CK(head_bwd(m, r, hin, g));
    for (int li = (int)m->layers.size() - 1; li >= 0; --li) {
        const Layer& L = m->layers[li];
        const void* lin = li > 0 ? layer_out(m, m->layers[li - 1]) : m->W(m->stem_out);
#define STEP(call) do { CK(call); void* _t = g; g = gn; gn = _t; } while (0)
        if (L.kind == Layer::CONV) { STEP(conv_bwd(m, m->convs[L.idx], r, lin, g, gn)); }
        else if (L.kind == Layer::SQZ) {
            SqzBlock& sb = m->sqz[L.idx];
            STEP(ffn_bwd(m, sb.ffn2, r, m->W(sb.conv.out), g, gn));
            STEP(sqzconv_bwd(m, sb.conv, r, m->W(sb.mha.out), g, gn));
            STEP(mhsa_bwd(m, sb.mha, r, m->W(sb.ffn1.out), g, gn));
// ... 169 lines not shown
```

ishara_amd/csrc/kernels.h:

```cpp
#pragma once
#include "common.h"
#include "../../include/ishara_hip.h"

enum DType : int { DT_F32 = 0, DT_BF16 = 1, DT_F16 = 2 };
static inline size_t dt_size(int dt) { return dt == DT_F32 ? 4 : 2; }
static inline bool dt_is16(int dt) { return dt != DT_F32; }

enum : int { OP_NONE = 0, OP_SWISH = 1, OP_COLAFFINE = 2, OP_ROWSCALE = 3, OP_DROPMASK = 4 };
struct OpArgs {
    const float* c1 = nullptr;
    const float* c0 = nullptr;
    const float* rs = nullptr;
    int T = 1;
    DropSpec drop = {0, 0, 1.f};
};

enum : int { ACT_NONE = 0, ACT_SWISH = 1, ACT_RELU = 2 };
enum : int { DACT_NONE = 0, DACT_SWISH = 1, DACT_POS = 2 };
enum : int { EPI_STD = 0, EPI_QKV = 1 };
struct EpiArgs {
    const float* bias = nullptr;
    const float* addtab = nullptr;
    int tab_period = 1;
    void* pre_out = nullptr;
    int act = ACT_NONE;
    DropSpec drop = {0, 0, 1.f};
    const float* rowscale = nullptr;
    int T = 1;
    int rowscale_bias = 0;
    int dact = DACT_NONE;
    const void* aux = nullptr;
    const void* resid = nullptr;
    int mode = EPI_STD;
    void* q = nullptr; void* k = nullptr; void* vt = nullptr;
    int H = 1, dh = 1;
    int dbg = 0;
    const float* ln_gamma = nullptr;
    const float* ln_beta = nullptr;
    float ln_eps = 0.f;
    float* ln_mean = nullptr;
    float* ln_rstd = nullptr;
    const float* pa_P = nullptr;
    const float* pa_Q = nullptr;
    void* pro_out = nullptr;
    int head_major = 1;
    int ldc = 0, n_valid = 0;
    int as_flags = -1;
};

int launch_gemm_nt(int dtA, int dtM, int dtC, int op, const void* A, const void* Bt, void* C,
                   int M, int N, int K, int ldb, const OpArgs& oa, const EpiArgs& ea, hipStream_t s);
enum NtRoute { NT_REFUSED, NT_AS_F16, NT_BIG, NT_CS, NT_AS, NT_TILE_T, NT_GLDS, NT_REG };
NtRoute gemm_nt_route(int dtA, int dtM, int dtC, int op, const void* A, int M, int N, int K, int ldb, const EpiArgs& ea);
const char* gemm_nt_kernel_name(int dtA, int dtM, int dtC, int op, const void* A, int M, int N, int K, int ldb, const EpiArgs& ea);
bool gemm_nt_as_applicable(int dtC, int M, int N, int K, int ldb, const EpiArgs& ea);
bool gemm_nt_as_prologue_ok(int dtA, int dtM, int dtC, int M, int N, int K, int ldb, const EpiArgs& ea);
const char* gemm_nt_as_name(int dtC, int K, const EpiArgs& ea, int M, int N);
int launch_gemm_nt_as(int dtC, const void* A, const void* Bt, void* C, int M, int N, int K, int ldb, const EpiArgs& ea, hipStream_t s);
int launch_gemm_nt_as_f16(int dtC, const void* A, const void* Bt, void* C, int M, int N, int K, int ldb, const EpiArgs& ea, hipStream_t s);
bool gemm_nt_cs_applicable(int dtC, int M, int N, int K, int ldb, const EpiArgs& ea);
const char* gemm_nt_cs_name(const EpiArgs& ea);
int launch_gemm_nt_cs(int dtC, const void* A, const void* Bt, void* C, int M, int N, int K, int ldb, const EpiArgs& ea, hipStream_t s);
bool gemm_nt_big_applicable(int dtA, int dtM, int dtC, int op, const void* A, int M, int N, int K, int ldb, const EpiArgs& ea);
int launch_gemm_nt_big(int dtA, int dtM, int dtC, int op, const void* A, const void* Bt, void* C, int M, int N, int K, int ldb, const EpiArgs& ea, hipStream_t s);

size_t gemm_tn_slab_floats(int M, int Ka, int Nb, int dtM);
#define RED_MAXJOBS 48
struct RedJob { const float* slab; float* out0; float* out1; size_t stride; int n0, n, splits, nb, nbv, first_block; };
struct RedSink { RedJob job[RED_MAXJOBS]; int njobs = 0; int nblocks = 0; };
extern RedSink* g_red_sink;
void launch_reduce_slabs(const float* slab, float* out, int n, int splits, size_t stride, hipStream_t s);
void launch_reduce_slabs2(const float* slab, float* out0, int n0, float* out1, int n1, int splits, size_t stride, hipStream_t s, int nb = 0, int nbv = 0);
bool reduce_cols_ok(const float* slab, const float* out0, const float* out1, int n0, int n, size_t stride);
bool reduce_sink_full();
int launch_reduce_flush(RedSink* sink, hipStream_t s);
bool gemm_tn_bias_rowscale_ok(int dtA, int dtB, int dtM, int M, int Ka, int Nb, int T);
struct TnDefer { float* slab[2] = {nullptr, nullptr}; int turn = 0; bool pending = false;
                 const float* p_slab = nullptr; float* p_out0 = nullptr; float* p_out1 = nullptr; int p_n0 = 0, p_n = 0, p_splits = 0; size_t p_stride = 0; int p_nb = 0, p_nbv = 0; };
int launch_gemm_tn_flush(TnDefer* defer, hipStream_t s);
struct TnPsa { const float* P = nullptr; const float* Q = nullptr;
               const void* W = nullptr; int ldw = 0;
               float* G = nullptr; float* Rpart = nullptr; int T = 0;
               int dbg = 0; };
bool gemm_tn_psa_ok(int dtA, int dtB, int dtM, int M, int Ka, int Nb, int T);
int launch_gemm_tn(int dtA, int dtB, int dtM, int opA, int opB, const void* A, const void* B,
                   float* out, float* dbias, float* slab, int M, int Ka, int Nb,
                   const OpArgs& oa, const OpArgs& ob, hipStream_t s, int ka_valid = 0, int nb_valid = 0,
                   const float* bias_rowscale = nullptr, int bias_T = 0, TnDefer* defer = nullptr, const TnPsa* psa = nullptr);
int launch_dense_narrow(int dt, const void* A, const void* Wt, int ldt, const float* bias, float* C, int M, int N, int K, hipStream_t s);
int launch_pack_rows_bf16(const float* x, void* xb, int M, int F, int Kp, hipStream_t s, int dt = DT_BF16);

enum TnRoute { TN_REFUSED, TN_BIG, TN_TR, TN_TR_BRS, TN_TR_PSA, TN_REG };
TnRoute gemm_tn_route(int dtA, int dtB, int dtM, int opA, int opB, int M, int Ka, int Nb, int ka_valid, int nb_valid, bool brs, int brsT, bool psa, int psaT);
const char* gemm_tn_kernel_name(int dtA, int dtB, int dtM, int opA, int opB, int M, int Ka, int Nb, int ka_valid = 0, int nb_valid = 0,
                                const float* bias_rowscale = nullptr, int bias_T = 0, const TnPsa* psa = nullptr);
int gemm_tn_big_plan(int M, int Ka, int Nb, int* splits_out);
int launch_gemm_tn_big(const void* A, const void* B, float* slab, int want_bias, int M, int Ka, int Nb, int* splits_out, const float* brs, int brsT, hipStream_t s);
extern int g_force_tn_regstage;
extern int g_force_regstage, g_dbg_tn, g_force_dw_lds, g_tn_blocks, g_attn_bwd_two_pass, g_as_flags_override, g_nt_big;
extern int g_tn_phase;

int launch_make_shadow(int dtM, const float* W, int K, int N, void* Wt, int ldt, void* Wn, int ldn, hipStream_t s);
struct ShadowDesc { const float* W; void* Wt; void* Wn; int K, N, ldt, ldn, tile0, tiles_n; };
int launch_make_shadow_batched(int dtM, const ShadowDesc* tab, int ntab, int total_tiles, hipStream_t s);

int launch_log_softmax_fwd(const float* x, float* y, int M, int C, int ld, hipStream_t s);
int launch_log_softmax_bwd(const float* dy, const float* y, float* dx, int M, int C, int ld, hipStream_t s);
int launch_layernorm_fwd(int dt, const void* x, const float* gamma, const float* beta, float eps,
                         void* y, float* mean, float* rstd, int M, int C, hipStream_t s);
size_t layernorm_bwd_scratch_floats(int C);
int launch_layernorm_bwd(int dt, const void* dy, const void* x, const float* mean, const float* rstd,
                         const float* gamma, const void* resid, void* dx, float* dgamma, float* dbeta,
                         float* scratch, int M, int C, hipStream_t s);

enum : int { DWIN_NONE = 0, DWIN_SWISH = 1, DWIN_GLU = 2 };
int launch_dwconv_fwd(int dt, int inop, const void* x, const float* w, const float* bias, void* y,
                      float* ssum, float* ssq, float* part, int B, int T, int C, int k, int padl, hipStream_t s, int* part_rows = nullptr);
size_t dwconv_fwd_scratch_floats(int B, int T, int C);
size_t dwconv_bwd_scratch_floats(int C, int k);
struct DwBnArgs { const void* h = nullptr; const float* mean = nullptr; const float* rstd = nullptr; const float* a = nullptr;
                  const float* sg = nullptr; const float* E = nullptr; const float* Fc = nullptr; int e_per_sample = 0; };
int launch_dwconv_bwd_bn(int dt, int inop, const void* dy, const DwBnArgs& bn, const void* x, const float* w, void* dx,
                         float* dw, float* dbias, float* scratch, int B, int T, int C, int k, int padl, hipStream_t s);
int launch_dwconv_bwd(int dt, int inop, const void* dy, const void* x, const float* w, void* dx,
                      float* dw, float* dbias, float* scratch, int B, int T, int C, int k, int padl, hipStream_t s);
bool dwconv_bwd_fused_ok(int dt, int C, int k, int padl);
int launch_dwconv_bwd_fused(int dt, int inop, const void* dy, const void* x, const float* w, void* dx, float* part,
                            int B, int T, int C, int k, int padl, int max_rows, hipStream_t s, const DwBnArgs& bn);

int launch_bn_finalize(const float* ssum, const float* ssq, int nb, float count, const float* gamma, const float* beta,
                       float eps, float momentum, float* moving_mean, float* moving_var, int training,
                       float* mean, float* rstd, float* a, float* b, int C, hipStream_t s, float var_corr = 1.f, int stride = 0);
int launch_eca_fwd(const float* gap, const float* a, const float* b, const float* w5, float invT,
                   float* gn, float* sgate, float* P, float* Q, int B, int C, hipStream_t s, float* rs = nullptr, DropSpec dp = {0, 0, 1.f}, int dp_fold = 0);
int launch_eca_fwd_part(const float* part, int prows, float* gap_out, const float* a, const float* b, const float* w5, float invT,
                        float* gn, float* sgate, float* P, float* Q, int B, int C, hipStream_t s, float* rs = nullptr, DropSpec dp = {0, 0, 1.f}, int dp_fold = 0);
int launch_eca_fwd_infer(const float* part, int prows, const float* mm, const float* mv, const float* gamma, const float* beta, float eps, const float* w5, float invT,
                         float* gn, float* sgate, float* P, float* Q, int B, int C, hipStream_t s);
int launch_sample_affine(int dt, const void* x, const float* P, const float* Q, const void* resid, void* y,
                         int B, int T, int C, hipStream_t s);
int launch_col_affine(int dt, const void* x, const float* a, const float* b, void* y, int M, int C, hipStream_t s);
enum : int { MAP_SWISH = 0, MAP_ROWSCALE = 1, MAP_DROPMASK = 2 };
int launch_map_rows(int dt, int op, const void* x, void* y, const float* rs, DropSpec drop, int M, int T, int C, hipStream_t s);
int launch_sample_reduce(int dt, const void* dy, const void* other, const float* mean, const float* rstd,
// ... 66 lines not shown
```

ishara_amd/csrc/model.hip:

```cpp
#include "model_types.h"
#include <algorithm>
#include <cmath>
#include <initializer_list>
#include <utility>
#include <stdlib.h>

static thread_local char g_err[1024] = "";
void ishara_set_error(const char* fmt, ...) {
    va_list ap;
    va_start(ap, fmt);
    vsnprintf(g_err, sizeof(g_err), fmt, ap);
    va_end(ap);
}
extern "C" const char* ishara_last_error(void) { return g_err; }

__global__ void fill_u32_kernel(uint32_t* p, size_t n, uint32_t v) {
    for (size_t i = (size_t)blockIdx.x * blockDim.x + threadIdx.x; i < n; i += (size_t)gridDim.x * blockDim.x) p[i] = v;
}
int launch_fill_u32(void* p, size_t n_words, uint32_t v, hipStream_t s) {
    if (n_words == 0) return 0;
    const int grid = (int)((n_words + 255) / 256 < 1024 ? (n_words + 255) / 256 : 1024);
    hipLaunchKernelGGL(fill_u32_kernel, dim3(grid), dim3(256), 0, s, (uint32_t*)p, n_words, v);
    return launch_rc();
}
// ... 157 lines not shown
    }
    return 0;
}

extern "C" int ishara_bind(ishara_model* m, float* params, float* grads, float* opt_m, float* opt_v, float* opt_slow, void* workspace, int64_t workspace_bytes) {
    if (!params || !workspace) { ishara_set_error("ishara_bind: params and workspace are required"); return -1; }
    if ((size_t)workspace_bytes < m->ws_need) { ishara_set_error("ishara_bind: workspace too small (%lld < %zu)", (long long)workspace_bytes, m->ws_need); return -1; }
    if (((uintptr_t)workspace) % 256 != 0) { ishara_set_error("ishara_bind: workspace must be 256-byte aligned"); return -1; }
    m->params = params; m->grads = grads; m->om = opt_m; m->ov = opt_v; m->oslow = opt_slow;
    m->ws = (char*)workspace; m->ws_bytes = workspace_bytes;
    m->shadow_ready = false;
    if (m->guard) {
        std::vector<uint32_t> pat(64, 0xA5C3A5C3u);
        for (size_t off : m->guard_offs) HIP_CHECK_RET(hipMemcpy(m->ws + off, pat.data(), 256, hipMemcpyHostToDevice));
    }
    if (m->family == ISHARA_FAMILY_TORCH_SQUEEZEFORMER) CK(r4_bind(m));
    if (m->family == ISHARA_FAMILY_KERAS_HYBRID) HIP_CHECK_RET(hipMemcpy(m->ws + m->pe.off, m->pe_host.data(), m->pe_host.size() * sizeof(float), hipMemcpyHostToDevice));
    return 0;
}

extern "C" int ishara_sync_weights(ishara_model* m, ishara_stream st) {
    hipStream_t s = (hipStream_t)st;
    if (!m->ws) { ishara_set_error("not bound"); return -1; }
    if (!m->shadow_ready) {
        HIP_CHECK_RET(hipMemsetAsync(m->ws + m->shadow_begin, 0, m->shadow_end - m->shadow_begin, s));
        if (m->guard) {
            static const std::vector<uint32_t> pat(64, 0xA5C3A5C3u);
            for (size_t off : m->guard_offs)
                if (off >= m->shadow_begin && off < m->shadow_end) HIP_CHECK_RET(hipMemcpyAsync(m->ws + off, pat.data(), 256, hipMemcpyHostToDevice, s));
        }
        std::vector<ShadowDesc> tab;
        int tile0 = 0;
        for (DenseW* w : m->denses) {
            ShadowDesc d;
            d.W = m->P(w->w); d.Wt = m->ws + w->wt; d.Wn = m->ws + w->wn; d.K = w->K; d.N = w->N; d.ldt = w->ldt; d.ldn = w->ldn;
            d.tile0 = tile0; d.tiles_n = (w->N + 31) / 32;
            tile0 += d.tiles_n * ((w->K + 31) / 32);
            tab.push_back(d);
        }
        m->shadow_tiles = tile0;
        m->shadow_ntab = (int)tab.size();
        m->shadow_tab_host = tab;
        HIP_CHECK_RET(hipMemcpyAsync(m->ws + m->shadow_tab_off, m->shadow_tab_host.data(), tab.size() * sizeof(ShadowDesc), hipMemcpyHostToDevice, s));
        m->shadow_ready = true;
    }
    CK(launch_make_shadow_batched(m->dt, reinterpret_cast<const ShadowDesc*>(m->ws + m->shadow_tab_off), m->shadow_ntab, m->shadow_tiles, s));
    return 0;
}

int gemm_fwd(ishara_model* m, const DenseW& w, const void* A, int dtA, void* Cc, int dtC, int M, int aop, const OpArgs& oa, EpiArgs ea) {
    if (w.b >= 0) ea.bias = m->P(w.b);
    const double by = (double)M * w.K * dt_size(dtA) + (double)M * w.N * dt_size(dtC) * (1 + (ea.resid ? 1 : 0) + (ea.pre_out ? 1 : 0)) + (double)w.K * w.N * dt_size(m->dt);
    CKP(m, gemm_nt_kernel_name(dtA, m->dt, dtC, aop, A, M, w.N, w.K, w.ldt, ea), by, 2.0 * M * w.N * w.K, launch_gemm_nt(dtA, m->dt, dtC, aop, A, m->ws + w.wt, Cc, M, w.N, w.K, w.ldt, oa, ea, m->s));
    return 0;
}
int gemm_dgrad(ishara_model* m, const DenseW& w, const void* dY, int dtA, void* dX, int M, int aop, const OpArgs& oa, const EpiArgs& ea) {
    const double by = (double)M * w.N * dt_size(dtA) + (double)M * w.K * dt_size(m->dt) * (1 + (ea.resid ? 1 : 0) + (ea.aux ? 1 : 0)) + (double)w.K * w.N * dt_size(m->dt);
    CKP(m, gemm_nt_kernel_name(dtA, m->dt, m->dt, aop, dY, M, w.K, w.N, w.ldn, ea), by, 2.0 * M * w.N * w.K, launch_gemm_nt(dtA, m->dt, m->dt, aop, dY, m->ws + w.wn, dX, M, w.K, w.N, w.ldn, oa, ea, m->s));
    return 0;
}
int red_flush(ishara_model* m) {
    if (m->red.njobs == 0) { m->red_off = 0; return 0; }
    CKP(m, "reduce_jobs(deferred)", 0, 0, launch_reduce_flush(&m->red, m->s));
    m->red_off = 0;
    return 0;
}
static float* red_scratch(ishara_model* m, size_t floats) {
    if (!m->red_on || floats > m->red_cap) return m->Wf(m->slab);
    floats = (floats + 63) & ~(size_t)63;
    if (m->red_off + floats > m->red_cap || reduce_sink_full()) { g_red_sink = nullptr; (void)red_flush(m); }
    g_red_sink = &m->red;
    float* p = m->Wf(m->red_arena) + m->red_off;
    m->red_off += floats;
    return p;
}
struct RedScope {
    ~RedScope() { g_red_sink = nullptr; }
};
int layernorm_bwd_deferred(ishara_model* m, const Run& r, const void* dy, const void* x, Buf mean, Buf rstd, const Norm& ln, const void* resid, void* dx) {
    RedScope scope;
    CKP(m, "layernorm_bwd", 4.0 * r.M * m->d * (double)dt_size(m->dt), 0, launch_layernorm_bwd(m->dt, dy, x, m->Wf(mean), m->Wf(rstd), m->P(ln.gamma), resid, dx, m->G(ln.gamma), m->G(ln.beta), red_scratch(m, layernorm_bwd_scratch_floats(m->d)), r.M, m->d, m->s));
    return 0;
}
int dwconv_bwd_deferred(ishara_model* m, const Run& r, double by_factor, int inop, const void* dy, const DwBnArgs* bn, const void* x, int dw, int dwb, void* dx, int C, int k, int padl) {
    RedScope scope;
    float* dbias = dwb >= 0 ? m->G(dwb) : nullptr;
    int fused = 0;
    if (bn) CKP(m, "dwconv_bwd", by_factor * r.M * m->d * (double)dt_size(m->dt), 0, (fused = launch_dwconv_bwd_bn(m->dt, inop, dy, *bn, x, m->P(dw), dx, m->G(dw), dbias, red_scratch(m, dwconv_bwd_scratch_floats(C, k)), r.B, m->T, C, k, padl, m->s)) < 0 ? fused : 0);
    else CKP(m, "dwconv_bwd", by_factor * r.M * m->d * (double)dt_size(m->dt), 0, launch_dwconv_bwd(m->dt, inop, dy, x, m->P(dw), dx, m->G(dw), dbias, red_scratch(m, dwconv_bwd_scratch_floats(C, k)), r.B, m->T, C, k, padl, m->s));
    return fused;
}
const void* grad_through_dropout(ishara_model* m, const Run& r, uint32_t site, float rate, const void* g, void* tmp, int T, int cols, int* rc) {
    const DropSpec od = dspec(r, site, rate);
    *rc = 0;
    if (!od.thr) return g;
    *rc = [&]() -> int {
        CKP(m, "map_rows", 2.0 * r.M * cols * (double)dt_size(m->dt), 0, launch_map_rows(m->dt, MAP_DROPMASK, g, tmp, nullptr, od, r.M, T, cols, m->s));
        return 0;
    }();
    return tmp;
}
int gemm_wgrad(ishara_model* m, const DenseW& w, const void* A, int dtA, int aop, const OpArgs& oa, const void* dY, int dtB, int bop, const OpArgs& ob, int M, int ka_valid, int nb_valid,
               const float* bias_rowscale, int bias_T, const TnPsa* psa) {
    const double by = (double)M * w.K * dt_size(dtA) + (double)M * w.N * dt_size(dtB) + (double)w.K * w.N * 4;
    if (m->tn_defer_on && !m->prof.on) {
        m->tn_defer.slab[0] = m->Wf(m->slab2[0]); m->tn_defer.slab[1] = m->Wf(m->slab2[1]);
        return launch_gemm_tn(dtA, dtB, m->dt, aop, bop, A, dY, m->G(w.w), w.b >= 0 ? m->G(w.b) : nullptr, m->Wf(m->slab), M, w.K, w.N, oa, ob, m->s, ka_valid, nb_valid, bias_rowscale, bias_T, &m->tn_defer, psa);
    }
    g_tn_phase = 1;
    CKP(m, gemm_tn_kernel_name(dtA, dtB, m->dt, aop, bop, M, w.K, w.N, ka_valid, nb_valid, bias_rowscale, bias_T, psa), by, 2.0 * M * w.N * w.K, launch_gemm_tn(dtA, dtB, m->dt, aop, bop, A, dY, m->G(w.w), w.b >= 0 ? m->G(w.b) : nullptr, m->Wf(m->slab), M, w.K, w.N, oa, ob, m->s, ka_valid, nb_valid, bias_rowscale, bias_T, nullptr, psa));
    g_tn_phase = 2;
    CKP(m, "reduce_slabs(wgrad)", 0, 0, launch_gemm_tn(dtA, dtB, m->dt, aop, bop, A, dY, m->G(w.w), w.b >= 0 ? m->G(w.b) : nullptr, m->Wf(m->slab), M, w.K, w.N, oa, ob, m->s, ka_valid, nb_valid, bias_rowscale, bias_T, nullptr, psa));
    g_tn_phase = 0;
    return 0;
}

int wgrad_flush(ishara_model* m) { return launch_gemm_tn_flush(&m->tn_defer, m->s); }

extern "C" int32_t ishara_grad_buckets(const ishara_model* m) { return (int32_t)m->bucket_lo.size(); }
extern "C" int ishara_grad_bucket(const ishara_model* m, int32_t i, int64_t* offset, int64_t* count) {
    if (i < 0 || i >= (int32_t)m->bucket_lo.size()) { ishara_set_error("ishara_grad_bucket: index %d outside 0..%d", i, (int)m->bucket_lo.size() - 1); return -1; }
    *offset = m->bucket_lo[i]; *count = m->bucket_hi[i] - m->bucket_lo[i];
    return 0;
}
extern "C" int ishara_grad_bucket_wait(ishara_model* m, int32_t i, ishara_stream side) {
    if (i < 0 || i >= (int32_t)m->bucket_lo.size()) { ishara_set_error("ishara_grad_bucket_wait: index %d outside 0..%d", i, (int)m->bucket_lo.size() - 1); return -1; }
    if (m->bucket_ev.empty()) { ishara_set_error("ishara_grad_bucket_wait: call ishara_grad_buckets_enable before the backward pass"); return -1; }
    HIP_CHECK_RET(hipStreamWaitEvent((hipStream_t)side, m->bucket_ev[i], 0));
    return 0;
}
extern "C" int ishara_grad_buckets_enable(ishara_model* m) {
    if (!m->bucket_ev.empty()) return 0;
    m->bucket_ev.resize(m->bucket_lo.size());
    for (auto& e : m->bucket_ev) HIP_CHECK_RET(hipEventCreateWithFlags(&e, hipEventDisableTiming));
    return 0;
}

static int optimizer_step(ishara_model* m, const char* who, float lr, float weight_decay, const float* grad, ishara_grad_stats* rec, int skip, ishara_stream st) {
    if (!m->om || !m->ov || !m->oslow || !m->grads) { ishara_set_error("%s: optimizer slots are not bound", who); return -1; }
    hipStream_t s = (hipStream_t)st;
    m->opt_iter += 1;
    const double t = (double)m->opt_iter, b1 = 0.9, b2 = 0.999;
    const double b1p = pow(b1, t), b2p = pow(b2, t);
    const double sma_inf = 2.0 / (1.0 - b2) - 1.0;
    const double sma_t = sma_inf - 2.0 * t * b2p / (1.0 - b2p);
    RAdamArgs a;
    a.lr = lr; a.wd = weight_decay; a.beta1 = (float)b1; a.beta2 = (float)b2; a.eps = 1e-7f;
    a.c1 = (float)(1.0 / (1.0 - b1p)); a.c2 = (float)(1.0 / (1.0 - b2p));
    a.rect = sma_t >= 4.0 ? 1 : 0;
    a.r_t = a.rect ? (float)sqrt(fmax((sma_t - 4.0) / (sma_inf - 4.0) * (sma_t - 2.0) / (sma_inf - 2.0) * sma_inf / sma_t, 0.0)) : 0.f;
    a.sync = (m->opt_iter % 5 == 0) ? 1 : 0;
    a.slow_step = 0.5f;
    m->s = s;
    if (!grad) grad = m->grads;
    if (rec) CKP(m, "radam_lookahead", 28.0 * m->n_train, 0, launch_radam_lookahead_ex(m->params, grad, m->om, m->ov, m->oslow, m->n_train, a, rec, skip, s));
    else CKP(m, "radam_lookahead", 28.0 * m->n_train, 0, launch_radam_lookahead(m->params, grad, m->om, m->ov, m->oslow, m->n_train, a, s));
    CKP(m, "weight_shadows", 0, 0, ishara_sync_weights(m, st));
    return 0;
}
extern "C" int ishara_optimizer_step(ishara_model* m, float lr, float weight_decay, ishara_stream st) {
    return optimizer_step(m, "ishara_optimizer_step", lr, weight_decay, nullptr, nullptr, 0, st);
}
extern "C" int ishara_optimizer_step_ex(ishara_model* m, float lr, float weight_decay, const float* grad, ishara_grad_stats* rec, int32_t skip_nonfinite,
                                        ishara_stream st) {
    const char* who = "ishara_optimizer_step_ex";
    if (!m) { ishara_set_error("%s: null handle", who); return -1; }
// ... 74 lines not shown
```

ishara_amd/csrc/model_types.h:

```cpp
#pragma once
#include <stdarg.h>
#include <stdio.h>
#include <string.h>
#include <math.h>
#include <string>
#include <vector>
#include <map>
#include "kernels.h"
#include "../../include/ishara_hip.h"

#define CK(expr) do { int _r = (expr); if (_r != 0) return _r; } while (0)
#define CKP(m, key, by, fl, expr)                                                          \
    do {                                                                                   \
        ProfRec* _pr = nullptr;                                                            \
        if ((m)->prof.on) {                                                                \
            (m)->prof.recs.push_back(ProfRec{key, (m)->prof.get(), (m)->prof.get(), (double)(by), (double)(fl)}); \
            _pr = &(m)->prof.recs.back();                                                  \
            (void)hipEventRecord(_pr->e0, (m)->s);                                         \
        }                                                                                  \
        int _r = (expr);                                                                   \
        if (_pr) (void)hipEventRecord(_pr->e1, (m)->s);                                    \
        if (_r != 0) return _r;                                                            \
    } while (0)

// ... 71 lines not shown
    int cls_pad = 0; Buf dlb;
    int stem_kp = 0; Buf stem_xb;
    Buf stem_h0, stem_out, stem_ssum, stem_ssq, stem_mean, stem_rstd, stem_a, stem_bsh, pe;
    std::vector<ConvBlock> convs;
    std::vector<SqzBlock> sqz;
    std::vector<ConfBlock> conf;
    std::vector<Layer> layers;
    int family = 0;
    std::vector<R5Block> r5; Buf r5_x, t4, fac;
    struct R4State* r4 = nullptr;
    DenseW topW, clsW; uint32_t head_site = 0; Buf head_hh;
    uint32_t nsites = 0;
    std::vector<DenseW*> denses;
    RedSink red; Buf red_arena; size_t red_cap = 0, red_off = 0; bool red_on = false;
    TnDefer tn_defer; Buf slab2[2]; bool tn_defer_on = false;
    Buf gA, gB, t1, t2, t3, S1, S2, E, Fc, Ecol, ecap, dse, dgapT, slab, ctcws, dlogits, nllb, delta;
    Buf psaG, psaR; bool psa_on = false;
    size_t shadow_begin = 0, shadow_end = 0;
    size_t shadow_tab_off = 0;
    std::vector<ShadowDesc> shadow_tab_host;
    int shadow_ntab = 0, shadow_tiles = 0;
    bool shadow_ready = false;
    size_t ws_need = 0;
    float* params = nullptr; float* grads = nullptr; float* om = nullptr; float* ov = nullptr; float* oslow = nullptr;
    char* ws = nullptr; int64_t ws_bytes = 0;
    std::vector<float> pe_host;
    int lastB = 0; int last_training = 0; uint32_t last_seed = 0; const float* last_x = nullptr;
    int opt_iter = 0;
    int probe_mod = -1, probe_B = 0; uint32_t probe_seed = 0;
    hipStream_t s = nullptr;

    int addp(const std::string& name, int64_t r, int64_t c, bool trainable) {
        ParamEntry e; e.name = name; e.ndim = c > 0 ? 2 : 1; e.shape[0] = r; e.shape[1] = c > 0 ? c : 0; e.offset = -1; e.trainable = trainable;
        entries.push_back(e);
        return (int)entries.size() - 1;
    }
    size_t cur = 0;
    bool guard = false; std::vector<size_t> guard_offs; std::vector<std::pair<size_t, size_t>> allocs;
    Buf alloc(size_t bytes) {
        Buf b; b.off = cur; cur = rup(cur + bytes, 256);
        allocs.push_back({b.off, bytes});
        if (guard) { guard_offs.push_back(cur); cur += 256; }
        return b;
    }
    Buf act(int cols) { return alloc((size_t)Bmax * T * cols * dt_size(dt)); }
    Buf f32(size_t n) { return alloc(n * sizeof(float)); }
    DenseW dense_named(const std::string& wname, const std::string& bname, int K, int N) {
        DenseW w; w.K = K; w.N = N;
        w.w = addp(wname, K, N, true);
        if (!bname.empty()) w.b = addp(bname, N, 0, true);
        return w;
    }
    DenseW dense(const std::string& name, int K, int N, bool bias) { return dense_named(name + "/kernel", bias ? name + "/bias" : "", K, N); }
    Norm norm(const std::string& name, int c) { Norm n; n.gamma = addp(name + "/gamma", c, 0, true); n.beta = addp(name + "/beta", c, 0, true); return n; }
    Norm norm_named(const std::string& prefix, int c) { Norm n; n.gamma = addp(prefix + ".weight", c, 0, true); n.beta = addp(prefix + ".bias", c, 0, true); return n; }
    BNp bnp(const std::string& name, int c) {
        BNp b; b.gamma = addp(name + "/gamma", c, 0, true); b.beta = addp(name + "/beta", c, 0, true);
        b.mm = addp(name + "/moving_mean", c, 0, false); b.mv = addp(name + "/moving_variance", c, 0, false);
        return b;
    }
    float* P(int idx) const { return params + entries[idx].offset; }
    float* G(int idx) const { return grads + entries[idx].offset; }
    template <typename TT = void> TT* W(Buf b) const { return reinterpret_cast<TT*>(ws + b.off); }
    float* Wf(Buf b) const { return reinterpret_cast<float*>(ws + b.off); }
};


struct Run { int B, M, training; uint32_t seed; };
static inline DropSpec dspec(const Run& r, uint32_t site, float rate) { return make_drop(r.seed, site, rate, r.training != 0); }
static inline DropSpec dspec_attn(const Run& r, uint32_t site, float rate) { return make_drop_attn(r.seed, site, rate, r.training != 0); }
void finish_param_layout(ishara_model* m);
void plan_shadow(ishara_model* m, DenseW& w, int min_ldt = 0, int min_ldn = 0);
void plan_confconv(ishara_model* m, ConfConv& c, size_t rows, int B, int d);
void plan_post_ln_ffn(ishara_model* m, R5FFN& f, size_t rows, int d, int de);
size_t wgrad_slab_floats(const ishara_model* m, size_t M, int min_K = 0);
size_t slab_floats(const ishara_model* m, size_t M, int B, int T, int maxw, int min_K = 0);
int gemm_fwd(ishara_model* m, const DenseW& w, const void* A, int dtA, void* Cc, int dtC, int M, int aop, const OpArgs& oa, EpiArgs ea);
int gemm_dgrad(ishara_model* m, const DenseW& w, const void* dY, int dtA, void* dX, int M, int aop, const OpArgs& oa, const EpiArgs& ea);
int gemm_wgrad(ishara_model* m, const DenseW& w, const void* A, int dtA, int aop, const OpArgs& oa, const void* dY, int dtB, int bop, const OpArgs& ob, int M, int ka_valid = 0, int nb_valid = 0,
               const float* bias_rowscale = nullptr, int bias_T = 0, const TnPsa* psa = nullptr);
int wgrad_flush(ishara_model* m);
int red_flush(ishara_model* m);
int layernorm_bwd_deferred(ishara_model* m, const Run& r, const void* dy, const void* x, Buf mean, Buf rstd, const Norm& ln, const void* resid, void* dx);
int dwconv_bwd_deferred(ishara_model* m, const Run& r, double by_factor, int inop, const void* dy, const DwBnArgs* bn, const void* x, int dw, int dwb, void* dx, int C, int k, int padl);
const void* grad_through_dropout(ishara_model* m, const Run& r, uint32_t site, float rate, const void* g, void* tmp, int T, int cols, int* rc);
void keras_build_graph(ishara_model* m);
void keras_plan_workspace(ishara_model* m);
bool ln_as_prologue(int dt, int M, int N, int K, int ldt, const float* gamma, const float* beta, float eps, float* mean, float* rstd, void* xn, EpiArgs& ea);
enum { CLS_AUTO = 0, CLS_AS = 1, CLS_NARROW = 2, CLS_GEMM = 3 };
int cls_route_auto(int dt, int M, int K, int C);
int classifier_fwd(ishara_model* m, int route, int dt, const void* A, const void* Wt, int ldt, const float* bias, float* logits, int M, int K, int C, hipStream_t s);
int confconv_fwd(ishara_model* m, ConfConv& c, const Run& r, const void* x);
int confconv_bwd(ishara_model* m, ConfConv& c, const Run& r, const void* x, const void* g, void* gn);
int r5_ffn_fwd(ishara_model* m, R5FFN& f, const Run& r, const void* x);
int r5_ffn_bwd(ishara_model* m, R5FFN& f, const Run& r, const void* x, const void* g, void* gn);
int r5_ln_fwd(ishara_model* m, const Run& r, const void* x, const Norm& n, void* y, Buf mean, Buf rstd);
int r5_ln_bwd(ishara_model* m, const Run& r, const void* g, const void* x, const Norm& n, Buf mean, Buf rstd, void* dx);
int r5_from_f32(int dt, const float* x, void* y, size_t n, hipStream_t s);
int r5_to_f32(int dt, const void* x, float* y, size_t n, hipStream_t s);
int r5_validate(const ishara_config& c);
void r5_build_graph(ishara_model* m);
void r5_plan_workspace(ishara_model* m);
int r4_validate(const ishara_config& c);
void r4_build_graph(ishara_model* m);
void r4_plan_workspace(ishara_model* m);
int r4_bind(ishara_model* m);
void r4_destroy(ishara_model* m);
int r4_output_frames(const ishara_model* m);
int r4_forward(ishara_model* m, const float* x, int32_t B, float* y, int32_t training, uint32_t seed, hipStream_t st);
int r4_backward(ishara_model* m, const float* dy, int32_t B, float* dx, hipStream_t st);
struct R4Dims { int T1, F1, T2, F2, T3, Fr, Kp; };
R4Dims r4_dims(int T0, int F, int d);
int launch_relattn_fwd(int dt, const void* q, const void* k, const void* v, const float* posp, const float* u, const float* vb, void* o, float* lse,
                       int B, int H, int T, int dh, float scale, DropSpec drop, hipStream_t s);
int launch_relattn_bwd(int dt, const void* q, const void* k, const void* v, const float* posp, const float* u, const float* vb, const void* o, const void* dO,
                       const float* lse, float* delta, void* dq, void* dk, void* dv, float* du, float* dvb, float* dposp,
                       int B, int H, int T, int dh, float scale, DropSpec drop, hipStream_t s);
int r4_subsample_fwd_launch(int dt, const float* x, const float* w1, const float* b1, const float* w2, const float* b2, float* y1, void* sub,
                            int B, int T0, int F, int d, int T1, int F1, int T2, int F2, hipStream_t s);
int r4_subsample_bwd_launch(int dt, const void* dsub, const void* sub, const float* y1, const float* x, const float* w1, const float* w2, float* dz1,
                            float* dw1, float* db1, float* dw2, float* db2, float* dx, int B, int T0, int F, int d, int T1, int F1, int T2, int F2, hipStream_t s);
int r4_tred_fwd_launch(int dt, const void* h, const float* w, const float* b, float* pre, void* out, int B, int Tin, int d, int Tr, int Fr, int Kp, hipStream_t s);
int r4_tred_wgrad_launch(int dt, const void* trout, const void* g, float* dwred, float* dW, float* db, float* slab, int M, int Fr, int Kp, int d, hipStream_t s);
int r4_tred_bwd_launch(int dt, const void* dout, const float* pre, const void* h, const float* w, const void* extra, float* dw, float* db, void* dh,
                       int B, int Tin, int d, int Tr, int Fr, int Kp, hipStream_t s);
int r4_rows_mode_launch(int dt, int mode, const void* src, const void* a, void* dst, int B, int Tdst, int Tsrc, int d, hipStream_t s);
int r4_fill_f32_launch(float* p, size_t n, float v, hipStream_t s);
```

Baseline: 7.059 million frames/s.

## Fuse LayerNorm backward into the A-stationary dgrad GEMM epilogue

Adds an LN-backward epilogue to the CS (A-stationary, K-streamed) GEMM kernel, so the dgrad GEMM that feeds a pre-LayerNorm computes dx, adds the residual gradient, and accumulates per-block dgamma/dbeta partials, which a small slab reduction then combines. The kernel is also generalised over the number of K stages (for example K=768 for the MHSA QKV dgrad). The FFN, MHSA and squeeze-conv backward paths route through this fused op when the CS route applies. This removes the intermediate dxn write/read and the separate layernorm_bwd launch, at the cost of higher register and LDS pressure in the GEMM tail and more complex wait scheduling.

```diff
diff --git a/include/ishara_hip.h b/include/ishara_hip.h
--- a/include/ishara_hip.h
+++ b/include/ishara_hip.h
@@ -125,6 +125,11 @@
                         float* out, ishara_stream s);
 
 int ishara_debug_set_as_flags(int32_t flags);
+int64_t ishara_debug_dgrad_layernorm_bwd_scratch_bytes(int32_t M, int32_t K);
+int ishara_debug_dgrad_layernorm_bwd(int32_t as_flags, const void* dy, const float* W, const void* x, const float* mean, const float* rstd,
+                                     const float* gamma, const void* resid, void* dxn, void* dx, float* dgamma, float* dbeta,
+                                     int32_t M, int32_t K, void* scratch, ishara_stream s);
+const char* ishara_debug_dgrad_layernorm_bwd_kernel_name(int32_t as_flags, int32_t M, int32_t K);
 const char* ishara_debug_dense_kernel_name(int32_t dt, int32_t M, int32_t K, int32_t N, int32_t act, int32_t with_resid);
 int ishara_debug_set_nt_big(int32_t on);
 int ishara_debug_force_regstage(int32_t on);
diff --git a/ishara_amd/_lib.py b/ishara_amd/_lib.py
--- a/ishara_amd/_lib.py
+++ b/ishara_amd/_lib.py
@@ -88,6 +88,9 @@
     "ishara_dropout_mask": (C.c_int, [_U32, _U32, _I32, _I32, _F, _P, _P]),
     "ishara_debug_set_as_flags": (C.c_int, [_I32]),
     "ishara_debug_dense_kernel_name": (C.c_char_p, [_I32, _I32, _I32, _I32, _I32, _I32]),
+    "ishara_debug_dgrad_layernorm_bwd_scratch_bytes": (C.c_int64, [_I32, _I32]),
+    "ishara_debug_dgrad_layernorm_bwd": (C.c_int, [_I32, _P, _P, _P, _P, _P, _P, _P, _P, _P, _P, _P, _I32, _I32, _P, _P]),
+    "ishara_debug_dgrad_layernorm_bwd_kernel_name": (C.c_char_p, [_I32, _I32, _I32]),
     "ishara_debug_set_nt_big": (C.c_int, [_I32]),
     "ishara_debug_force_regstage": (C.c_int, [_I32]),
     "ishara_debug_module_count": (_I32, [_P]),
diff --git a/ishara_amd/csrc/api_ops.hip b/ishara_amd/csrc/api_ops.hip
--- a/ishara_amd/csrc/api_ops.hip
+++ b/ishara_amd/csrc/api_ops.hip
@@ -189,6 +189,50 @@
     const void* aligned = reinterpret_cast<const void*>(uintptr_t(256));
     EpiArgs ea; ea.bias = reinterpret_cast<const float*>(aligned); ea.act = act; ea.resid = with_resid ? aligned : nullptr; ea.dbg = g_dbg_epi;
     return gemm_nt_kernel_name(dt, dt, dt, OP_NONE, aligned, M, N, K, sh.ldt, ea);
+}
+static size_t dgrad_lnb_partial_floats(int M) { return std::max(layernorm_bwd_scratch_floats(256), (size_t)gemm_nt_cs_lnb_rows(M) * 512); }
+extern "C" int64_t ishara_debug_dgrad_layernorm_bwd_scratch_bytes(int32_t M, int32_t K) {
+    if (M < 1 || K < 1) return -1;
+    return (int64_t)(OpShadow(DT_BF16, 256, K, M).slab + dgrad_lnb_partial_floats(M) * sizeof(float));
+}
+static EpiArgs dgrad_lnb_epi(int as_flags, const void* x, const float* mean, const float* rstd, const float* gamma, const void* resid, float* partial) {
+    EpiArgs ea; ea.as_flags = as_flags; ea.resid = resid;
+    ea.lnb_x = x; ea.lnb_mean = mean; ea.lnb_rstd = rstd; ea.lnb_gamma = gamma; ea.lnb_partial = partial;
+    return ea;
+}
+extern "C" int ishara_debug_dgrad_layernorm_bwd(int32_t as_flags, const void* dy, const float* Wm, const void* x, const float* mean, const float* rstd,
+                                                const float* gamma, const void* resid, void* dxn, void* dx, float* dgamma, float* dbeta,
+                                                int32_t M, int32_t K, void* scratch, ishara_stream st) {
+    const char* me = "ishara_debug_dgrad_layernorm_bwd";
+    if (M < 1 || K < 8 || K % 8) { ishara_set_error("%s: M=%d K=%d unsupported", me, M, K); return -1; }
+    if (!dy || !Wm || !x || !mean || !rstd || !gamma || !resid || !dxn || !dx || !dgamma || !dbeta || !scratch) { ishara_set_error("%s: null argument", me); return -1; }
+    hipStream_t s = (hipStream_t)st;
+    const int dt = DT_BF16, d = 256;
+    const OpShadow sh(dt, d, K, M);
+    char* sc = (char*)scratch;
+    CK(sh.build(dt, Wm, d, K, sc, s));
+    float* partial = reinterpret_cast<float*>(sc + sh.slab);
+    OpArgs no;
+    const EpiArgs ea = dgrad_lnb_epi(as_flags, x, mean, rstd, gamma, resid, partial);
+    if (gemm_nt_route(dt, dt, dt, OP_NONE, dy, M, d, K, sh.ldn, ea) == NT_CS) {
+        CK(launch_gemm_nt(dt, dt, dt, OP_NONE, dy, sc + sh.wn, dx, M, d, K, sh.ldn, no, ea, s));
+        launch_reduce_slabs2(partial, dgamma, d, dbeta, d, gemm_nt_cs_lnb_rows(M), (size_t)2 * d, s);
+        return launch_rc();
+    }
+    EpiArgs e0; e0.as_flags = as_flags;
+    CK(launch_gemm_nt(dt, dt, dt, OP_NONE, dy, sc + sh.wn, dxn, M, d, K, sh.ldn, no, e0, s));
+    return launch_layernorm_bwd(dt, dxn, x, mean, rstd, gamma, resid, dx, dgamma, dbeta, partial, M, d, s);
+}
+extern "C" const char* ishara_debug_dgrad_layernorm_bwd_kernel_name(int32_t as_flags, int32_t M, int32_t K) {
+    if (M < 1 || K < 8 || K % 8) return "";
+    const int dt = DT_BF16, d = 256;
+    const OpShadow sh(dt, d, K, M);
+    const void* aligned = reinterpret_cast<const void*>(uintptr_t(256));
+    const float* fa = reinterpret_cast<const float*>(aligned);
+    const EpiArgs ea = dgrad_lnb_epi(as_flags, aligned, fa, fa, fa, aligned, const_cast<float*>(fa));
+    if (gemm_nt_route(dt, dt, dt, OP_NONE, aligned, M, d, K, sh.ldn, ea) == NT_CS) return gemm_nt_kernel_name(dt, dt, dt, OP_NONE, aligned, M, d, K, sh.ldn, ea);
+    EpiArgs e0; e0.as_flags = as_flags;
+    return gemm_nt_kernel_name(dt, dt, dt, OP_NONE, aligned, M, d, K, sh.ldn, e0);
 }
 extern "C" int ishara_op_dense_bwd(int32_t dt, const void* x, const float* Wm, const void* dy, void* dx, float* dW, float* db,
                                    int32_t M, int32_t K, int32_t N, void* scratch, ishara_stream st) {
diff --git a/ishara_amd/csrc/gemm_cs.hip b/ishara_amd/csrc/gemm_cs.hip
--- a/ishara_amd/csrc/gemm_cs.hip
+++ b/ishara_amd/csrc/gemm_cs.hip
@@ -1,6 +1,7 @@
 #include <cstdio>
 #include <cstdlib>
 #include <map>
+#include <type_traits>
 #include "common.h"
 #include "kernels.h"
 
@@ -13,6 +14,8 @@
 #define CS_STAGE 32768
 #define CS_DPW 4
 #define CS_LDS (CS_RING * CS_STAGE + CS_N * 4 + 2 * CS_K * 4)
+#define CS_K12 768
+#define CS_LNB_LDS (CS_LDS + CS_N * 4 + 8 * 2 * CS_N * 4)
 #define CS_DEFAULT_FLAGS 115
 #define CS_MIN_M 49153
 
@@ -51,11 +54,11 @@
     int mrow[RT];
     cs_u32x4 a[3][RT][2];
 };
-template <int RT> DEVI void cs_rows_init(CsRows<RT>& r, const bf16* __restrict__ A, int M, int mw, const CsLane& L) {
+template <int RT, int NST> DEVI void cs_rows_init(CsRows<RT>& r, const bf16* __restrict__ A, int M, int mw, const CsLane& L) {
 #pragma unroll
     for (int i = 0; i < RT; ++i) {
         r.mrow[i] = min(mw + 16 * i + L.c, M - 1);
-        r.ap[i] = A + (size_t)r.mrow[i] * CS_K + L.g * 8;
+        r.ap[i] = A + (size_t)r.mrow[i] * (64 * NST) + L.g * 8;
     }
 }
 template <int RT, int S> DEVI void cs_load_a(CsRows<RT>& r) {
@@ -83,19 +86,22 @@
 }
 #define CS_PREFETCH_OPS(RT) (2 * 2 * (RT) + 3 * CS_DPW)
 
-template <int MASK, int PRO, int RT, int E, int S>
+template <int MASK, int PRO, int RT, int E, int S, int NST, bool LATE>
 DEVI void cs_stage(CsRows<RT>& r, const CsLane& L, char* smem, const float* pq_s, f32x4 (&acc)[8][2][RT], bf16* pro_out, int M, int mw,
                    bool full, bool pout, bool nt_side) {
     constexpr int NA = 2 * RT, D = CS_DPW;
-    if constexpr (S == 0) cs_wait<2 * D + E, 2 * D + E>(full, pout);
+    static_assert(!LATE || PRO == 0, "no prologue row stores with the late A request");
+    if constexpr (S == 0 && LATE) cs_wait<NA + E, NA + E>(full, pout);
+    else if constexpr (S == 1 && LATE) cs_wait<D + E + NA, D + E + NA>(full, pout);
+    else if constexpr (S == 0) cs_wait<2 * D + E, 2 * D + E>(full, pout);
     else if constexpr (S == 1) cs_wait<2 * D + E + NA, 2 * D + E + NA + NA>(full, pout);
-    else if constexpr (S <= 5) cs_wait<2 * D + NA, 2 * D + NA + 2 * NA>(full, pout);
-    else if constexpr (S == 6) cs_wait<D + NA, D + NA + 2 * NA>(full, pout);
+    else if constexpr (S <= NST - 3) cs_wait<2 * D + NA, 2 * D + NA + 2 * NA>(full, pout);
+    else if constexpr (S == NST - 2) cs_wait<D + NA, D + NA + 2 * NA>(full, pout);
     else cs_wait<0, 2 * NA>(full, pout);
     asm volatile("s_waitcnt lgkmcnt(0)" ::: "memory");
     __builtin_amdgcn_s_barrier();
-    if constexpr (S + 2 < CS_NST) cs_load_a<RT, S + 2>(r);
-    if constexpr (S + 3 < CS_NST) cs_issue_w<S + 3>(L, smem);
+    if constexpr (S + 2 < NST) cs_load_a<RT, S + 2>(r);
+    if constexpr (S + 3 < NST) cs_issue_w<S + 3>(L, smem);
     constexpr int B = S % 3;
 #pragma unroll
     for (int i = 0; i < RT; ++i) { cs_pin(r.a[B][i][0]); cs_pin(r.a[B][i][1]); }
@@ -140,9 +146,165 @@
     }
 }
 
-template <int MASK, int PRO, int RT, int E, typename HAND>
+template <int P, int NP, typename F> DEVI void cs_for(F&& f) {
+    if constexpr (P < NP) { f(std::integral_constant<int, P>{}); cs_for<P + 1, NP>(f); }
+}
+
+struct CsLnb {
+    const bf16* x;
+    const float* gam_s;
+    const float* mean; const float* rstd;
+    float* slot;
+};
+DEVI float cs_ld4(const float* p) {
+    float r;
+    asm volatile("global_load_dword %0, %1, off" : "=v"(r) : "v"(p) : "memory");
+    return r;
+}
+DEVI void cs_pin(float& r) { asm volatile("" : "+v"(r)); }
+DEVI float cs_mul_r(float a, float b) {
+#pragma clang fp contract(off)
+    return a * b;
+}
+DEVI float cs_row16_sum(float v) {
+    v += __builtin_bit_cast(float, __builtin_amdgcn_update_dpp(0, __builtin_bit_cast(int, v), 0x128, 0xf, 0xf, true));
+    v += __builtin_bit_cast(float, __builtin_amdgcn_update_dpp(0, __builtin_bit_cast(int, v), 0x124, 0xf, 0xf, true));
+    v += __builtin_bit_cast(float, __builtin_amdgcn_update_dpp(0, __builtin_bit_cast(int, v), 0x122, 0xf, 0xf, true));
+    v += __builtin_bit_cast(float, __builtin_amdgcn_update_dpp(0, __builtin_bit_cast(int, v), 0x121, 0xf, 0xf, true));
+    return v;
+}
+typedef __attribute__((address_space(3))) f32x4 cs_lds_f4;
+DEVI uint32_t cs_lds_off(const void* p) { return (uint32_t)(uintptr_t)(__attribute__((address_space(3))) const void*)p; }
+DEVI void cs_lds8(uint32_t off, float (&v)[8]) {
+    const f32x4 a = *(cs_lds_f4*)(uintptr_t)off, b = *(cs_lds_f4*)(uintptr_t)(off + 16);
+#pragma unroll
+    for (int e = 0; e < 4; ++e) { v[e] = a[e]; v[4 + e] = b[e]; }
+}
+DEVI void cs_lds8_st(uint32_t off, const float (&v)[8]) {
+    *(cs_lds_f4*)(uintptr_t)off = f32x4{v[0], v[1], v[2], v[3]};
+    *(cs_lds_f4*)(uintptr_t)(off + 16) = f32x4{v[4], v[5], v[6], v[7]};
+}
+template <int RT, bool FIRST, typename HAND>
+DEVI void cs_lnb_tail(f32x4 (&acc)[8][2][RT], const CsRows<RT>& r, const CsLane& L, bf16* __restrict__ C, int M, const EpiArgs& ea, CsLnb& ln,
+                      int mw, bool full, int hops, HAND hand) {
+    uint32_t gam = cs_lds_off(ln.gam_s + 8 * L.g), slot = cs_lds_off(ln.slot + 8 * L.g);
+    asm volatile("" : "+v"(gam), "+v"(slot));
+    cs_u32x4 dn[RT][8];
+#pragma unroll
+    for (int i = 0; i < RT; ++i)
+#pragma unroll
+        for (int p = 0; p < 8; ++p) { asm volatile("" : "+v"(acc[p][0][i])); asm volatile("" : "+v"(acc[p][1][i])); }
+#pragma unroll
+    for (int i = 0; i < RT; ++i)
+#pragma unroll
+        for (int p = 0; p < 8; ++p) {
+            bf16x8 t;
+#pragma unroll
+            for (int e = 0; e < 4; ++e) { t[e] = (bf16)acc[p][0][i][e]; t[4 + e] = (bf16)acc[p][1][i][e]; }
+            dn[i][p] = __builtin_bit_cast(cs_u32x4, t);
+            if (!full && mw + 16 * i + L.c >= M) dn[i][p] = cs_u32x4{0u, 0u, 0u, 0u};
+            cs_pin(dn[i][p]);
+        }
+    const bf16* xp[RT];
+    const bf16* gp[RT];
+    bf16* cp[RT];
+    auto rows_of = [&](auto ic) {
+        constexpr int i = decltype(ic)::value;
+        int mr = r.mrow[i];
+        asm volatile("" : "+v"(mr));
+        const size_t eoff = (size_t)mr * CS_N + 8 * L.g;
+        xp[i] = ln.x + eoff;
+        gp[i] = reinterpret_cast<const bf16*>(ea.resid) + eoff;
+        cp[i] = C + eoff;
+    };
+    rows_of(std::integral_constant<int, 0>{});
+    cs_u32x4 xs[RT][8], gs[RT][8];
+    float mus[RT], rss[RT];
+    mus[0] = cs_ld4(ln.mean + r.mrow[0]);
+    rss[0] = cs_ld4(ln.rstd + r.mrow[0]);
+    cs_for<0, 8>([&](auto pc) { constexpr int p = decltype(pc)::value; xs[0][p] = cs_ld16<64 * p>(xp[0]); });
+    cs_for<0, 8>([&](auto pc) { constexpr int p = decltype(pc)::value; gs[0][p] = cs_ld16<64 * p>(gp[0]); });
+    asm volatile("s_waitcnt lgkmcnt(0)" ::: "memory");
+    __builtin_amdgcn_s_barrier();
+    hand(std::integral_constant<int, 0>{});
+    if (hops) cs_wait_vm<3 * CS_DPW>(); else cs_wait_vm<0>();
+    cs_for<0, RT>([&](auto ic) {
+        constexpr int i = decltype(ic)::value;
+        if constexpr (i > 0) cs_wait_vm<0>();
+#pragma unroll
+        for (int p = 0; p < 8; ++p) { cs_pin(xs[i][p]); cs_pin(gs[i][p]); }
+        cs_pin(mus[i]); cs_pin(rss[i]);
+        if constexpr (i == RT - 1) hand(std::integral_constant<int, 1>{});
+        const float mu = mus[i], rsd = rss[i];
+        float s1p[8], s2p[8];
+#pragma unroll
+        for (int p = 0; p < 8; ++p) {
+            float ga[8], dv[8], xv[8], cg[8], cb[8];
+            if (p > 0) { cs_pin(s1p[p - 1]); cs_pin(s2p[p - 1]); }
+            cs_lds8(gam + 128 * p, ga);
+            cs_unpack(dn[i][p], dv);
+            cs_unpack(xs[i][p], xv);
+            float a1 = 0.f, a2 = 0.f;
+#pragma unroll
+            for (int e = 0; e < 8; ++e) {
+                const float xh = cs_mul_r(xv[e] - mu, rsd);
+                cg[e] = cs_mul_r(dv[e], xh);
+                cb[e] = dv[e];
+                const float d = cs_mul_r(dv[e], ga[e]);
+                a1 += d;
+                a2 += cs_mul_r(d, xh);
+            }
+            a1 += __shfl_xor(a1, 16); a1 += __shfl_xor(a1, 32);
+            a2 += __shfl_xor(a2, 16); a2 += __shfl_xor(a2, 32);
+            s1p[p] = a1; s2p[p] = a2;
+#pragma unroll
+            for (int e = 0; e < 8; ++e) cg[e] = cs_row16_sum(cg[e]);
+            cs_pin(s1p[p]); cs_pin(s2p[p]);
+#pragma unroll
+            for (int e = 0; e < 8; ++e) cb[e] = cs_row16_sum(cb[e]);
+            if (L.c == p) {
+                const uint32_t sp = slot + 128 * p;
+                if (!(FIRST && i == 0)) {
+                    float og[8], ob[8];
+                    cs_lds8(sp, og); cs_lds8(sp + 4 * CS_N, ob);
+#pragma unroll
+                    for (int e = 0; e < 8; ++e) { cg[e] += og[e]; cb[e] += ob[e]; }
+                }
+                cs_lds8_st(sp, cg);
+                cs_lds8_st(sp + 4 * CS_N, cb);
+            }
+        }
+        const float s1 = (((s1p[0] + s1p[1]) + (s1p[2] + s1p[3])) + ((s1p[4] + s1p[5]) + (s1p[6] + s1p[7]))) * (1.f / CS_N);
+        const float s2 = (((s2p[0] + s2p[1]) + (s2p[2] + s2p[3])) + ((s2p[4] + s2p[5]) + (s2p[6] + s2p[7]))) * (1.f / CS_N);
+        const bool valid = full || mw + 16 * i + L.c < M;
+        cs_for<0, 8>([&](auto pc) {
+            constexpr int p = decltype(pc)::value;
+            float ga[8], dv[8], xv[8], o[8];
+            cs_pin(dn[i][p]); cs_pin(xs[i][p]);
+            cs_lds8(gam + 128 * p, ga);
+            cs_unpack(dn[i][p], dv);
+            cs_unpack(xs[i][p], xv);
+            cs_unpack(gs[i][p], o);
+#pragma unroll
+            for (int e = 0; e < 8; ++e) {
+                const float xh = cs_mul_r(xv[e] - mu, rsd);
+                const float t = __builtin_fmaf(-s2, xh, cs_mul_r(dv[e], ga[e]) - s1);
+                o[e] = __builtin_fmaf(rsd, t, o[e]);
+            }
+            if (valid) store8(cp[i] + 32 * p, o);
+            if constexpr (i + 1 < RT) {
+                if constexpr (p == 0) { rows_of(std::integral_constant<int, i + 1>{}); mus[i + 1] = cs_ld4(ln.mean + r.mrow[i + 1]); rss[i + 1] = cs_ld4(ln.rstd + r.mrow[i + 1]); }
+                xs[i + 1][p] = cs_ld16<64 * p>(xp[i + 1]);
+                gs[i + 1][p] = cs_ld16<64 * p>(gp[i + 1]);
+            }
+        });
+    });
+}
+
+template <int MASK, int PRO, int RT, int E, int NST, int LNB, typename HAND>
 DEVI void cs_pass(CsRows<RT>& r, const CsLane& L, bf16* __restrict__ C, int M, const EpiArgs& ea, char* smem, const float* bias_s, const float* pq_s,
-                  int m_base, float rsc, int hops, HAND hand) {
+                  int m_base, float rsc, int hops, CsLnb* ln, HAND hand) {
+    static_assert(PRO == 0 || NST == CS_NST, "the per-sample affine's P, Q rows are laid out for K = 512");
     const int mw = m_base + L.wid * 16 * RT;
     const bool full = m_base + 128 * RT <= M;
     const bool pout = PRO != 0 && ea.pro_out != nullptr;
@@ -150,16 +312,10 @@
     constexpr bool f_resid = (MASK & CS_RESID) != 0, f_drop = (MASK & CS_DROP) != 0, f_rowscale = (MASK & CS_ROWSCALE) != 0;
     f32x4 acc[8][2][RT];
     bf16* po = reinterpret_cast<bf16*>(ea.pro_out);
-    cs_stage<MASK, PRO, RT, E, 0>(r, L, smem, pq_s, acc, po, M, mw, full, pout, nt_side);
-    cs_stage<MASK, PRO, RT, E, 1>(r, L, smem, pq_s, acc, po, M, mw, full, pout, nt_side);
-    cs_stage<MASK, PRO, RT, E, 2>(r, L, smem, pq_s, acc, po, M, mw, full, pout, nt_side);
-    cs_stage<MASK, PRO, RT, E, 3>(r, L, smem, pq_s, acc, po, M, mw, full, pout, nt_side);
-    cs_stage<MASK, PRO, RT, E, 4>(r, L, smem, pq_s, acc, po, M, mw, full, pout, nt_side);
-    cs_stage<MASK, PRO, RT, E, 5>(r, L, smem, pq_s, acc, po, M, mw, full, pout, nt_side);
-    cs_stage<MASK, PRO, RT, E, 6>(r, L, smem, pq_s, acc, po, M, mw, full, pout, nt_side);
-    cs_stage<MASK, PRO, RT, E, 7>(r, L, smem, pq_s, acc, po, M, mw, full, pout, nt_side);
+    cs_for<0, NST>([&](auto sc) { cs_stage<MASK, PRO, RT, E, decltype(sc)::value, NST, LNB == 2>(r, L, smem, pq_s, acc, po, M, mw, full, pout, nt_side); });
 
     asm volatile("s_nop 15");
+    if constexpr (LNB != 0) { cs_lnb_tail<RT, LNB == 1>(acc, r, L, C, M, ea, *ln, mw, full, hops, hand); return; }
     size_t eoff[RT];
 #pragma unroll
     for (int i = 0; i < RT; ++i) eoff[i] = (size_t)r.mrow[i] * CS_N + 8 * L.g;
@@ -175,7 +331,7 @@
     }
     asm volatile("s_waitcnt lgkmcnt(0)" ::: "memory");
     __builtin_amdgcn_s_barrier();
-    hand();
+    if constexpr (LNB == 0) hand();
     if constexpr (f_resid) {
         if (hops) cs_wait_vm<CS_PREFETCH_OPS(1)>(); else cs_wait_vm<0>();
 #pragma unroll
@@ -218,6 +374,24 @@
             store8(C + eoff[i] + 32 * p, v);
         }
     }
+}
+
+DEVI void cs_bsrc_init(CsLane& L, const bf16* __restrict__ Bt, int ldb, int lane) {
+#pragma unroll
+    for (int t = 0; t < CS_DPW; ++t) {
+        const int rr = (L.wid * CS_DPW + t) * 8 + (lane >> 3), p = lane & 7;
+        L.bsrc[t] = Bt + (size_t)rr * ldb + ((p ^ cs_swz(rr)) << 3);
+    }
+}
+DEVI void cs_lane_init(CsLane& L, const bf16* __restrict__ Bt, int ldb, int tid) {
+    const int lane = tid & 63;
+    L.wid = __builtin_amdgcn_readfirstlane(tid >> 6);
+    L.c = lane & 15; L.g = lane >> 4;
+    cs_bsrc_init(L, Bt, ldb, lane);
+    const int frow = 8 * (L.c >> 2) + (L.c & 3);
+    const int sx = L.g ^ cs_swz(frow);
+    L.off0 = frow * 128 + (sx << 4);
+    L.off1 = frow * 128 + ((sx ^ 4) << 4);
 }
 
 template <int MASK, int PRO>
@@ -225,7 +399,7 @@
     extern __shared__ __attribute__((aligned(16))) char cs_smem[];
     float* bias_s = reinterpret_cast<float*>(cs_smem + CS_RING * CS_STAGE);
     float* pq_s = bias_s + CS_N;
-    const int tid = threadIdx.x, lane = tid & 63;
+    const int tid = threadIdx.x;
     const int m_base = blockIdx.x * CS_ROWS;
     const int bsm = min(m_base, M - 1) / max(ea.T, 1);
     for (int n = tid; n < CS_N; n += 512) bias_s[n] = ea.bias ? ea.bias[n] : 0.f;
@@ -240,30 +414,90 @@
     asm volatile("" : "+v"(rsc));
 
     CsLane L;
-    L.wid = __builtin_amdgcn_readfirstlane(tid >> 6);
-    L.c = lane & 15; L.g = lane >> 4;
-#pragma unroll
-    for (int t = 0; t < CS_DPW; ++t) {
-        const int rr = (L.wid * CS_DPW + t) * 8 + (lane >> 3), p = lane & 7;
-        L.bsrc[t] = Bt + (size_t)rr * ldb + ((p ^ cs_swz(rr)) << 3);
-    }
-    const int frow = 8 * (L.c >> 2) + (L.c & 3);
-    const int sx = L.g ^ cs_swz(frow);
-    L.off0 = frow * 128 + (sx << 4);
-    L.off1 = frow * 128 + ((sx ^ 4) << 4);
+    cs_lane_init(L, Bt, ldb, tid);
 
     const bool two = m_base + 256 < M;
     CsRows<2> r1;
     CsRows<1> r2;
-    cs_rows_init<2>(r1, A, M, m_base + L.wid * 32, L);
+    cs_rows_init<2, CS_NST>(r1, A, M, m_base + L.wid * 32, L);
     cs_prefetch<2>(r1, L, cs_smem);
-    cs_pass<MASK, PRO, 2, 0>(r1, L, C, M, ea, cs_smem, bias_s, pq_s, m_base, rsc, two ? CS_PREFETCH_OPS(1) : 0, [&]() {
+    cs_pass<MASK, PRO, 2, 0, CS_NST, 0>(r1, L, C, M, ea, cs_smem, bias_s, pq_s, m_base, rsc, two ? CS_PREFETCH_OPS(1) : 0, nullptr, [&]() {
         if (two) {
-            cs_rows_init<1>(r2, A, M, m_base + 256 + L.wid * 16, L);
+            cs_rows_init<1, CS_NST>(r2, A, M, m_base + 256 + L.wid * 16, L);
             cs_prefetch<1>(r2, L, cs_smem);
         }
     });
-    if (two) cs_pass<MASK, PRO, 1, 16>(r2, L, C, M, ea, cs_smem, bias_s, pq_s, m_base + 256, rsc, 0, []() {});
+    if (two) cs_pass<MASK, PRO, 1, 16, CS_NST, 0>(r2, L, C, M, ea, cs_smem, bias_s, pq_s, m_base + 256, rsc, 0, nullptr, []() {});
+}
+
+__global__ __launch_bounds__(512, 1) void gemm_nt_cs12_kernel(const bf16* __restrict__ A, const bf16* __restrict__ Bt, bf16* __restrict__ C, int M, int ldb, EpiArgs ea) {
+    extern __shared__ __attribute__((aligned(16))) char cs_smem[];
+    float* bias_s = reinterpret_cast<float*>(cs_smem + CS_RING * CS_STAGE);
+    const int tid = threadIdx.x;
+    const int m_base = blockIdx.x * CS_ROWS;
+    for (int n = tid; n < CS_N; n += 512) bias_s[n] = ea.bias ? ea.bias[n] : 0.f;
+    __syncthreads();
+    CsLane L;
+    cs_lane_init(L, Bt, ldb, tid);
+    const bool two = m_base + 256 < M;
+    CsRows<2> r1;
+    CsRows<1> r2;
+    cs_rows_init<2, 12>(r1, A, M, m_base + L.wid * 32, L);
+    cs_prefetch<2>(r1, L, cs_smem);
+    cs_pass<0, 0, 2, 0, 12, 0>(r1, L, C, M, ea, cs_smem, bias_s, bias_s, m_base, 1.f, two ? CS_PREFETCH_OPS(1) : 0, nullptr, [&]() {
+        if (two) {
+            cs_rows_init<1, 12>(r2, A, M, m_base + 256 + L.wid * 16, L);
+            cs_prefetch<1>(r2, L, cs_smem);
+        }
+    });
+    if (two) cs_pass<0, 0, 1, 16, 12, 0>(r2, L, C, M, ea, cs_smem, bias_s, bias_s, m_base + 256, 1.f, 0, nullptr, []() {});
+}
+
+template <int NST>
+__global__ __launch_bounds__(512, 1) void gemm_nt_cs_lnb_kernel(const bf16* __restrict__ A, const bf16* __restrict__ Bt, bf16* __restrict__ C, int M, int ldb, EpiArgs ea) {
+    extern __shared__ __attribute__((aligned(16))) char cs_smem[];
+    float* gam_s = reinterpret_cast<float*>(cs_smem + CS_LDS);
+    float* col_s = gam_s + CS_N;
+    const int tid = threadIdx.x;
+    const int m_base = blockIdx.x * CS_ROWS;
+    for (int n = tid; n < CS_N; n += 512) gam_s[n] = ea.lnb_gamma[n];
+    CsLane L;
+    cs_lane_init(L, Bt, ldb, tid);
+    CsLnb ln;
+    ln.x = reinterpret_cast<const bf16*>(ea.lnb_x);
+    ln.gam_s = gam_s;
+    ln.slot = col_s + L.wid * (2 * CS_N);
+    ln.mean = ea.lnb_mean; ln.rstd = ea.lnb_rstd;
+    __syncthreads();
+
+    const bool two = m_base + 256 < M;
+    CsRows<2> r1;
+    CsRows<1> r2;
+    cs_rows_init<2, NST>(r1, A, M, m_base + L.wid * 32, L);
+    cs_prefetch<2>(r1, L, cs_smem);
+    cs_pass<CS_RESID, 0, 2, 0, NST, 1>(r1, L, C, M, ea, cs_smem, gam_s, gam_s, m_base, 1.f, two ? 3 * CS_DPW : 0, &ln, [&](auto phase) {
+        if (!two) return;
+        if constexpr (decltype(phase)::value == 0) {
+            cs_issue_w<0>(L, cs_smem);
+            cs_issue_w<1>(L, cs_smem);
+            cs_issue_w<2>(L, cs_smem);
+        } else {
+            cs_rows_init<1, NST>(r2, A, M, m_base + 256 + L.wid * 16, L);
+            cs_load_a<1, 0>(r2);
+            cs_load_a<1, 1>(r2);
+            int lane = L.c + 16 * L.g;
+            asm volatile("" : "+v"(lane));
+            cs_bsrc_init(L, Bt, ldb, lane);
+        }
+    });
+    if (two) cs_pass<CS_RESID, 0, 1, 8, NST, 2>(r2, L, C, M, ea, cs_smem, gam_s, gam_s, m_base + 256, 1.f, 0, &ln, [](auto) {});
+
+    __syncthreads();
+    float a = 0.f;
+    const int t = 64 * L.wid + 16 * L.g + L.c;
+#pragma unroll
+    for (int w = 0; w < 8; ++w) a += col_s[w * (2 * CS_N) + t];
+    ea.lnb_partial[(size_t)blockIdx.x * (2 * CS_N) + t] = a;
 }
 
 static int cs_mask_of(const EpiArgs& ea) {
@@ -275,16 +509,23 @@
     return ea.as_flags >= 0 ? ea.as_flags : (g_as_flags_override >= 0 ? g_as_flags_override : v);
 }
 bool gemm_nt_cs_applicable(int dtC, int M, int N, int K, int ldb, const EpiArgs& ea) {
-    if (dtC != DT_BF16 || K != CS_K || N != CS_N || M < 1 || ldb < CS_K || ldb % 8 != 0) return false;
+    if (dtC != DT_BF16 || (K != CS_K && K != CS_K12) || N != CS_N || M < 1 || ldb < K || ldb % 8 != 0) return false;
     const int flags = cs_flags(ea);
     if (!(flags & 64)) return false;
     if (ea.n_valid || ea.dbg || (ea.ldc && ea.ldc != CS_N) || ea.ln_gamma) return false;
     if (!(flags & 128) && M < CS_MIN_M) return false;
+    if (K == CS_K12 && !(flags & 512)) return false;
     const int mask = cs_mask_of(ea);
+    if (ea.lnb_x)
+        return (flags & 256) && mask == CS_RESID && !ea.bias && !ea.pa_P && ea.lnb_mean && ea.lnb_rstd && ea.lnb_gamma && ea.lnb_partial;
+    if (K == CS_K12) return mask == 0 && !ea.pa_P;
     if (ea.pa_P) return ea.pa_Q && ea.T > 0 && ea.T % CS_ROWS == 0 && (mask == CS_RESID || mask == (CS_RESID | CS_ROWSCALE));
     return mask == 0 || mask == CS_RESID || mask == (CS_RESID | CS_DROP);
 }
-const char* gemm_nt_cs_name(const EpiArgs& ea) {
+int gemm_nt_cs_lnb_rows(int M) { return (M + CS_ROWS - 1) / CS_ROWS; }
+const char* gemm_nt_cs_name(int K, const EpiArgs& ea) {
+    if (ea.lnb_x) return K == CS_K12 ? "gemm_nt_cs_lnb_kernel<12>" : "gemm_nt_cs_lnb_kernel<8>";
+    if (K == CS_K12) return "gemm_nt_cs12_kernel";
     static std::map<int, std::string> names;
     const int mask = cs_mask_of(ea), pro = ea.pa_P ? 2 : 0;
     auto it = names.find(mask | pro << 8);
@@ -295,6 +536,13 @@
     }
     return it->second.c_str();
 }
+template <typename KERN>
+static int cs_launch_k(KERN kern, int lds, const void* A, const void* Bt, void* C, int M, int ldb, const EpiArgs& ea, hipStream_t s, int& ready) {
+    if (!ready) ready = hipFuncSetAttribute(reinterpret_cast<const void*>(kern), hipFuncAttributeMaxDynamicSharedMemorySize, lds) == hipSuccess ? 1 : -1;
+    if (ready < 0) { ishara_set_error("gemm_nt_cs: %d bytes of LDS refused", lds); return -1; }
+    hipLaunchKernelGGL(kern, dim3((M + CS_ROWS - 1) / CS_ROWS), dim3(512), lds, s, (const bf16*)A, (const bf16*)Bt, (bf16*)C, M, ldb, ea);
+    return launch_rc();
+}
 template <int MASK, int PRO>
 static int cs_launch(const void* A, const void* Bt, void* C, int M, int ldb, const EpiArgs& ea, hipStream_t s) {
     static int ready = 0;
@@ -308,6 +556,10 @@
     EpiArgs ea = ea_in;
     ea.as_flags = cs_flags(ea_in);
     const int mask = cs_mask_of(ea);
+    static int ready[3] = {0, 0, 0};
+    if (ea.lnb_x) return K == CS_K12 ? cs_launch_k(gemm_nt_cs_lnb_kernel<12>, CS_LNB_LDS, A, Bt, C, M, ldb, ea, s, ready[0])
+                                     : cs_launch_k(gemm_nt_cs_lnb_kernel<8>, CS_LNB_LDS, A, Bt, C, M, ldb, ea, s, ready[1]);
+    if (K == CS_K12) return cs_launch_k(gemm_nt_cs12_kernel, CS_LDS, A, Bt, C, M, ldb, ea, s, ready[2]);
     if (ea.pa_P) return mask == CS_RESID ? cs_launch<CS_RESID, 2>(A, Bt, C, M, ldb, ea, s) : cs_launch<CS_RESID | CS_ROWSCALE, 2>(A, Bt, C, M, ldb, ea, s);
     if (mask == 0) return cs_launch<0, 0>(A, Bt, C, M, ldb, ea, s);
     if (mask == CS_RESID) return cs_launch<CS_RESID, 0>(A, Bt, C, M, ldb, ea, s);
diff --git a/ishara_amd/csrc/gemm_nt.hip b/ishara_amd/csrc/gemm_nt.hip
--- a/ishara_amd/csrc/gemm_nt.hip
+++ b/ishara_amd/csrc/gemm_nt.hip
@@ -519,16 +519,18 @@
 
 NtRoute gemm_nt_route(int dtA, int dtM, int dtC, int op, const void* A, int M, int N, int K, int ldb, const EpiArgs& ea) {
     const bool pro = ea.ln_gamma || ea.pa_P;
-    if (dtM == DT_F16) {
+    if (dtM == DT_F16 && !ea.lnb_x) {
         if (op != OP_NONE) return NT_REFUSED;
         if (dtA == DT_F16 && g_force_regstage == 0 && (K == 256 || K == 512) && ldb % 64 == 0 && ((uintptr_t)A) % 16 == 0 && gemm_nt_as_applicable(dtC, M, N, K, ldb, ea)) return NT_AS_F16;
         if (pro) return NT_REFUSED;
         return (dtA == DT_F16 && (dtC == DT_F16 || dtC == DT_F32)) || (dtA == DT_F32 && dtC == DT_F16) ? NT_REG : NT_REFUSED;
     }
     if (pro && (op != OP_NONE || !gemm_nt_as_prologue_ok(dtA, dtM, dtC, M, N, K, ldb, ea))) return NT_REFUSED;
-    if (g_force_regstage == 0 && gemm_nt_big_applicable(dtA, dtM, dtC, op, A, M, N, K, ldb, ea)) return NT_BIG;
+    if (ea.lnb_x && dtM != DT_BF16) return NT_REFUSED;
+    if (!ea.lnb_x && g_force_regstage == 0 && gemm_nt_big_applicable(dtA, dtM, dtC, op, A, M, N, K, ldb, ea)) return NT_BIG;
     const int bk = dtM == DT_BF16 ? 32 : 16;
     const bool dma_ok = op == OP_NONE && dtA == dtM && K % bk == 0 && ldb % (2 * bk) == 0 && ((uintptr_t)A) % 16 == 0;
+    if (ea.lnb_x) return dma_ok && g_force_regstage == 0 && dtM == DT_BF16 && !pro && gemm_nt_cs_applicable(dtC, M, N, K, ldb, ea) ? NT_CS : NT_REFUSED;
     if (dma_ok && g_force_regstage == 0 && dtM == DT_BF16 && gemm_nt_cs_applicable(dtC, M, N, K, ldb, ea)) return NT_CS;
     if (dma_ok && g_force_regstage == 0 && dtM == DT_BF16 && gemm_nt_as_applicable(dtC, M, N, K, ldb, ea)) return NT_AS;
     const bool dma_dt = (dtM == DT_F32 && dtC == DT_F32) || (dtM == DT_BF16 && (dtC == DT_BF16 || dtC == DT_F32));
@@ -555,6 +557,7 @@
             if (f16m && op != OP_NONE) ishara_set_error("gemm_nt: f16 operands take no operand transform");
             else if (f16m && (ea.ln_gamma || ea.pa_P)) ishara_set_error("gemm_nt: f16 operand prologue on a shape the A-stationary kernel does not take");
             else if (f16m) ishara_set_error("gemm_nt: unsupported f16 dtype combination %d/%d/%d", dtA, dtM, dtC);
+            else if (ea.lnb_x) ishara_set_error("gemm_nt: LayerNorm-backward epilogue requested for a call the C-stationary kernel does not take (check gemm_nt_cs_applicable first)");
             else if (ea.ln_gamma || ea.pa_P) ishara_set_error("gemm_nt: operand prologue requested for a shape the A-stationary kernel does not take (check gemm_nt_as_prologue_ok first)");
             else ishara_set_error("gemm_nt: unsupported dtype combination %d/%d/%d op %d", dtA, dtM, dtC, op);
             return -1;
@@ -584,7 +587,7 @@
     if (dtM == DT_F16) return "gemm_nt_kernel<f16>";
     switch (route) {
         case NT_BIG: return "gemm_nt_big_kernel<bf16>";
-        case NT_CS: return gemm_nt_cs_name(ea);
+        case NT_CS: return gemm_nt_cs_name(K, ea);
         case NT_AS: return gemm_nt_as_name(dtC, K, ea, M, N);
         case NT_TILE_T: return dtM == DT_F32 ? "gemm_nt_t_kernel<f32,f32>" : (dtC == DT_F32 ? "gemm_nt_t_kernel<bf16,f32>" : "gemm_nt_t_kernel<bf16,bf16>");
         case NT_GLDS: return dtM == DT_F32 ? "gemm_nt_glds_kernel<f32,f32>" : (dtC == DT_F32 ? "gemm_nt_glds_kernel<bf16,f32>" : "gemm_nt_glds_kernel<bf16,bf16>");
diff --git a/ishara_amd/csrc/keras_hybrid.hip b/ishara_amd/csrc/keras_hybrid.hip
--- a/ishara_amd/csrc/keras_hybrid.hip
+++ b/ishara_amd/csrc/keras_hybrid.hip
@@ -504,10 +504,8 @@
     EpiArgs e1; e1.drop = dspec(r, f.site_in, m->cfg.dropout_rate); e1.dact = DACT_SWISH; e1.aux = m->W(f.za);
     CK(gemm_dgrad(m, f.Wb, gs, dt, m->W(m->t1), r.M, OP_NONE, no, e1));
     CK(gemm_wgrad(m, f.Wb, m->W(f.u), dt, OP_NONE, no, gs, dt, OP_NONE, no, r.M));
-    EpiArgs e0;
-    CK(gemm_dgrad(m, f.Wa, m->W(m->t1), dt, m->W(m->t2), r.M, OP_NONE, no, e0));
     CK(gemm_wgrad(m, f.Wa, m->W(f.xn), dt, OP_NONE, no, m->W(m->t1), dt, OP_NONE, no, r.M));
-    return layernorm_bwd_deferred(m, r, m->W(m->t2), x, f.mean, f.rstd, f.ln, g, gn);
+    return dgrad_layernorm_bwd(m, r, f.Wa, m->W(m->t1), m->W(m->t2), x, f.mean, f.rstd, f.ln, g, gn);
 }
 
 static int mhsa_bwd(ishara_model* m, MHSA& a, const Run& r, const void* x, const void* g, void* gn) {
@@ -521,14 +519,13 @@
     const float scale = 1.0f / sqrtf((float)m->d);
     CKP(m, "attn_bwd", 8.0 * r.M * m->d * (double)dt_size(m->dt), 10.0 * r.B * m->H * (double)m->T * m->T * m->dh, launch_attn_bwd(dt, m->W(a.q), m->W(a.k), m->W(a.vt), m->W(a.o), m->W(m->t1), m->Wf(a.lse), m->Wf(m->delta), m->W(m->t2),
                        r.B, m->H, m->T, m->dh, scale, dspec_attn(r, a.site_attn, a.rate), 1, m->cfg.attn_impl, attn_maskw(m, a.maskw), m->s));
-    CK(gemm_dgrad(m, a.Wqkv, m->W(m->t2), dt, m->W(m->t1), r.M, OP_NONE, no, e0));
     CK(gemm_wgrad(m, a.Wqkv, m->W(a.xn), dt, OP_NONE, no, m->W(m->t2), dt, OP_NONE, no, r.M));
-    return layernorm_bwd_deferred(m, r, m->W(m->t1), x, a.mean, a.rstd, a.ln, g, gn);
+    return dgrad_layernorm_bwd(m, r, a.Wqkv, m->W(m->t2), m->W(m->t1), x, a.mean, a.rstd, a.ln, g, gn);
 }
 
 static int sqzconv_bwd(ishara_model* m, SqzConv& c, const Run& r, const void* x, const void* g, void* gn) {
     const int dt = m->dt, d = m->d, de = c.Wc1.N, B = r.B, T = m->T;
-    OpArgs no; EpiArgs e0;
+    OpArgs no;
     CKP(m, "sample_reduce", 2.0 * r.M * m->d * (double)dt_size(m->dt), 0, launch_sample_reduce(dt, g, m->W(c.u3), nullptr, nullptr, m->Wf(m->S1), m->Wf(m->dse), B, T, d, m->s));
     CKP(m, "se_bwd", 0, 0, launch_se_bwd(m->Wf(m->dse), m->Wf(c.gap), 1.f / T, m->P(c.seW1), m->P(c.seW2), m->Wf(c.hid), m->Wf(c.se),
                      m->G(c.seW1), m->G(c.seb1), m->G(c.seW2), m->G(c.seb2), m->Wf(m->dgapT), m->Wf(m->E), B, d, c.R, m->s));
@@ -537,9 +534,8 @@
     CK(gemm_dgrad(m, c.Wc3, m->W(m->t1), dt, m->W(m->t2), r.M, OP_NONE, no, e1));
     CK(gemm_wgrad(m, c.Wc3, m->W(c.hd), dt, OP_NONE, no, m->W(m->t1), dt, OP_NONE, no, r.M));
     CK(dwconv_bwd_deferred(m, r, 8.0, DWIN_SWISH, m->W(m->t2), nullptr, m->W(c.zc), c.dw, -1, m->W(m->t1), de, c.k, c.k - 1));
-    CK(gemm_dgrad(m, c.Wc1, m->W(m->t1), dt, m->W(m->t2), r.M, OP_NONE, no, e0));
     CK(gemm_wgrad(m, c.Wc1, m->W(c.xn), dt, OP_NONE, no, m->W(m->t1), dt, OP_NONE, no, r.M));
-    return layernorm_bwd_deferred(m, r, m->W(m->t2), x, c.mean, c.rstd, c.ln, g, gn);
+    return dgrad_layernorm_bwd(m, r, c.Wc1, m->W(m->t1), m->W(m->t2), x, c.mean, c.rstd, c.ln, g, gn);
 }
 
 int confconv_bwd(ishara_model* m, ConfConv& c, const Run& r, const void* x, const void* g, void* gn) {
diff --git a/ishara_amd/csrc/kernels.h b/ishara_amd/csrc/kernels.h
--- a/ishara_amd/csrc/kernels.h
+++ b/ishara_amd/csrc/kernels.h
@@ -46,6 +46,9 @@
     int head_major = 1;
     int ldc = 0, n_valid = 0;
     int as_flags = -1;
+    const void* lnb_x = nullptr;
+    const float* lnb_mean = nullptr; const float* lnb_rstd = nullptr; const float* lnb_gamma = nullptr;
+    float* lnb_partial = nullptr;
 };
 
 int launch_gemm_nt(int dtA, int dtM, int dtC, int op, const void* A, const void* Bt, void* C,
@@ -59,7 +62,8 @@
 int launch_gemm_nt_as(int dtC, const void* A, const void* Bt, void* C, int M, int N, int K, int ldb, const EpiArgs& ea, hipStream_t s);
 int launch_gemm_nt_as_f16(int dtC, const void* A, const void* Bt, void* C, int M, int N, int K, int ldb, const EpiArgs& ea, hipStream_t s);
 bool gemm_nt_cs_applicable(int dtC, int M, int N, int K, int ldb, const EpiArgs& ea);
-const char* gemm_nt_cs_name(const EpiArgs& ea);
+const char* gemm_nt_cs_name(int K, const EpiArgs& ea);
+int gemm_nt_cs_lnb_rows(int M);
 int launch_gemm_nt_cs(int dtC, const void* A, const void* Bt, void* C, int M, int N, int K, int ldb, const EpiArgs& ea, hipStream_t s);
 bool gemm_nt_big_applicable(int dtA, int dtM, int dtC, int op, const void* A, int M, int N, int K, int ldb, const EpiArgs& ea);
 int launch_gemm_nt_big(int dtA, int dtM, int dtC, int op, const void* A, const void* Bt, void* C, int M, int N, int K, int ldb, const EpiArgs& ea, hipStream_t s);
diff --git a/ishara_amd/csrc/model.hip b/ishara_amd/csrc/model.hip
--- a/ishara_amd/csrc/model.hip
+++ b/ishara_amd/csrc/model.hip
@@ -263,6 +263,28 @@
     CKP(m, "layernorm_bwd", 4.0 * r.M * m->d * (double)dt_size(m->dt), 0, launch_layernorm_bwd(m->dt, dy, x, m->Wf(mean), m->Wf(rstd), m->P(ln.gamma), resid, dx, m->G(ln.gamma), m->G(ln.beta), red_scratch(m, layernorm_bwd_scratch_floats(m->d)), r.M, m->d, m->s));
     return 0;
 }
+int dgrad_layernorm_bwd(ishara_model* m, const Run& r, const DenseW& w, const void* dY, void* dxn, const void* x, Buf mean, Buf rstd, const Norm& ln, const void* resid, void* gn) {
+    OpArgs no;
+    EpiArgs ea;
+    ea.resid = resid;
+    ea.lnb_x = x; ea.lnb_mean = m->Wf(mean); ea.lnb_rstd = m->Wf(rstd); ea.lnb_gamma = m->P(ln.gamma);
+    ea.lnb_partial = m->Wf(m->slab);
+    const bool fused = resid && m->dt == DT_BF16 && w.K == m->d && ((uintptr_t)dY) % 16 == 0 &&
+                       gemm_nt_route(m->dt, m->dt, m->dt, OP_NONE, dY, r.M, w.K, w.N, w.ldn, ea) == NT_CS;
+    if (!fused) {
+        EpiArgs e0;
+        CK(gemm_dgrad(m, w, dY, m->dt, dxn, r.M, OP_NONE, no, e0));
+        return layernorm_bwd_deferred(m, r, dxn, x, mean, rstd, ln, resid, gn);
+    }
+    RedScope scope;
+    const int rows = gemm_nt_cs_lnb_rows(r.M);
+    ea.lnb_partial = red_scratch(m, (size_t)rows * 2 * m->d);
+    const double s = (double)dt_size(m->dt);
+    CKP(m, gemm_nt_kernel_name(m->dt, m->dt, m->dt, OP_NONE, dY, r.M, w.K, w.N, w.ldn, ea), (double)r.M * w.N * s + 3.0 * r.M * m->d * s, 2.0 * r.M * w.N * w.K,
+        launch_gemm_nt(m->dt, m->dt, m->dt, OP_NONE, dY, m->ws + w.wn, gn, r.M, w.K, w.N, w.ldn, no, ea, m->s));
+    launch_reduce_slabs2(ea.lnb_partial, m->G(ln.gamma), m->d, m->G(ln.beta), m->d, rows, (size_t)2 * m->d, m->s);
+    return launch_rc();
+}
 int dwconv_bwd_deferred(ishara_model* m, const Run& r, double by_factor, int inop, const void* dy, const DwBnArgs* bn, const void* x, int dw, int dwb, void* dx, int C, int k, int padl) {
     RedScope scope;
     float* dbias = dwb >= 0 ? m->G(dwb) : nullptr;
diff --git a/ishara_amd/csrc/model_types.h b/ishara_amd/csrc/model_types.h
--- a/ishara_amd/csrc/model_types.h
+++ b/ishara_amd/csrc/model_types.h
@@ -177,6 +177,7 @@
 int wgrad_flush(ishara_model* m);
 int red_flush(ishara_model* m);
 int layernorm_bwd_deferred(ishara_model* m, const Run& r, const void* dy, const void* x, Buf mean, Buf rstd, const Norm& ln, const void* resid, void* dx);
+int dgrad_layernorm_bwd(ishara_model* m, const Run& r, const DenseW& w, const void* dY, void* dxn, const void* x, Buf mean, Buf rstd, const Norm& ln, const void* resid, void* gn);
 int dwconv_bwd_deferred(ishara_model* m, const Run& r, double by_factor, int inop, const void* dy, const DwBnArgs* bn, const void* x, int dw, int dwb, void* dx, int C, int k, int padl);
 const void* grad_through_dropout(ishara_model* m, const Run& r, uint32_t site, float rate, const void* g, void* tmp, int T, int cols, int* rc);
 void keras_build_graph(ishara_model* m);
```

Result: no change. 7.090 million frames/s, median of 6 (+0.4%).
